# jonassibbesen/rpvg

Measured on AMD Instinct MI355X. Metric: read-pairs quantified/sec, higher is better.
Workload: dtype f64

## Files before the change

### include/rpvg_hip.h

```cpp
#ifndef RPVG_HIP_H
#define RPVG_HIP_H

#include <stdint.h>

#include "rpvg_batch.h"
#include "rpvg_rows.h"
#include "rpvg_index.h"
#include "rpvg_table.h"
#include "rpvg_samples.h"
#include "rpvg_text.h"

#ifdef __cplusplus
extern "C" {
#endif

typedef enum rpvg_hip_status {
    RPVG_HIP_OK = 0,
    RPVG_HIP_ERR_NO_DEVICE = -1,
    RPVG_HIP_ERR_RUNTIME = -2,
    RPVG_HIP_ERR_INVALID = -3,
    RPVG_HIP_ERR_ALLOC = -4,
    RPVG_HIP_ERR_UNSUPPORTED = -5
} rpvg_hip_status;

// ... 241 lines not shown
    const double * abundances;
    const double * noise_count;
    const double * total_count;
    const uint32_t * iterations;
    const uint32_t * set_count;
    const double * cluster_noise_count;
    const uint32_t * set_size;
    const uint32_t * set_member;
    const double * set_posterior;
    const double * set_abundance;
    const uint32_t * sample_count;
    const uint64_t * words_consumed;
    const uint32_t * generator_state;
} rpvg_hip_subset_em_independent_view;

typedef struct rpvg_independent_limits {
    uint32_t max_group_size;
    uint32_t max_samples;
    uint64_t max_transcript_sets;
    uint32_t words_per_draw;
    uint32_t state_words;
    uint64_t max_work_bytes;
} rpvg_independent_limits;

typedef struct rpvg_hip_independent_stats {
    uint64_t calls_completed;
    uint64_t draws;
    uint64_t subsets;
} rpvg_hip_independent_stats;

int rpvg_hip_nested_independent_subset_em(rpvg_hip_ctx * ctx, const rpvg_hip_batch * batch, const rpvg_hip_groups * groups,
                                          const rpvg_hip_independent_spec * spec, rpvg_hip_subset_em ** result_out);
int rpvg_hip_subset_em_get_independent(const rpvg_hip_subset_em * result, rpvg_hip_subset_em_independent_view * view_out);
int rpvg_hip_independent_draws_get(const rpvg_hip_subset_em * result, uint32_t unit, uint32_t * draws_out);
void rpvg_hip_independent_limits(rpvg_independent_limits * limits_out);
int rpvg_hip_independent_stats_get(rpvg_hip_ctx * ctx, rpvg_hip_independent_stats * stats_out);

int rpvg_hip_min_path_cover(rpvg_hip_ctx * ctx, const rpvg_hip_batch * batch, uint32_t num_clusters,
                            const uint32_t * clusters, const uint64_t * cover_off, uint32_t * cover, uint32_t * cover_size);
int rpvg_hip_min_path_cover_any(rpvg_hip_ctx * ctx, const rpvg_hip_batch * batch, uint32_t num_clusters,
                                const uint32_t * clusters, const uint64_t * cover_off, uint32_t * cover, uint32_t * cover_size,
                                uint64_t grid_min_work, uint32_t * choice_order);
typedef struct rpvg_cover_limits {
    uint32_t workgroup_max_paths;
    uint32_t chunk_rounds;
    uint64_t default_grid_min_work;
    uint64_t grid_max_rows;
    uint64_t grid_max_entries;
    uint32_t pick_block;
    uint32_t pick_per_thread;
    uint32_t pick_max_blocks;
    uint32_t strike_block;
    uint32_t strike_max_blocks;
    uint32_t hist_max_paths;
} rpvg_cover_limits;
void rpvg_hip_cover_limits(rpvg_cover_limits * limits_out);

int rpvg_hip_path_clusters(rpvg_hip_ctx * ctx, uint32_t num_paths, uint64_t num_sets, const uint64_t * set_off,
                           const uint32_t * set_path, uint32_t * path_to_cluster, uint32_t * num_clusters_out,
                           uint64_t * cluster_off, uint32_t * cluster_paths);

typedef struct rpvg_hip_alignments rpvg_hip_alignments;
typedef struct rpvg_hip_read_rows rpvg_hip_read_rows;
int rpvg_hip_alignments_upload(rpvg_hip_ctx * ctx, const rpvg_alignment_batch * alignments, rpvg_hip_alignments ** out);
void rpvg_hip_alignments_free(rpvg_hip_ctx * ctx, rpvg_hip_alignments * alignments);
int rpvg_hip_read_rows_build(rpvg_hip_ctx * ctx, const rpvg_hip_alignments * alignments, const rpvg_row_params * params,
                             int32_t merge, rpvg_hip_read_rows ** rows_out);
int rpvg_hip_read_rows_to_batch(rpvg_hip_ctx * ctx, const rpvg_hip_read_rows * rows, rpvg_hip_batch ** batch_out);
int rpvg_hip_read_rows_sizes(rpvg_hip_ctx * ctx, const rpvg_hip_read_rows * rows, rpvg_cluster_batch * view);
int rpvg_hip_read_rows_view(rpvg_hip_ctx * ctx, rpvg_hip_read_rows * rows, rpvg_cluster_batch * view, double * build_ms,
                            double * merge_ms);
void rpvg_hip_read_rows_free(rpvg_hip_ctx * ctx, rpvg_hip_read_rows * rows);

int rpvg_hip_frag_length_fit(rpvg_hip_ctx * ctx, const uint32_t * counts, uint32_t n, int skew_normal, rpvg_frag_length_fit * out);
int rpvg_hip_frag_length_table(rpvg_hip_ctx * ctx, double loc, double scale, double shape, rpvg_hip_frag_table ** out);
int rpvg_hip_frag_length_table_get(rpvg_hip_ctx * ctx, const rpvg_hip_frag_table * table, double * log_prob_out);
void rpvg_hip_frag_length_table_free(rpvg_hip_ctx * ctx, rpvg_hip_frag_table * table);
int rpvg_hip_effective_lengths(rpvg_hip_ctx * ctx, double loc, double scale, double shape, const uint32_t * path_length, uint64_t n,
                               double * out);
int rpvg_hip_alignments_set_effective_lengths(rpvg_hip_ctx * ctx, rpvg_hip_alignments * alignments, double loc, double scale,
                                              double shape, const uint32_t * path_length, double * out);
int rpvg_hip_frag_length_eval(rpvg_hip_ctx * ctx, int what, const double * rows, uint64_t n, double * out);

int rpvg_hip_align_index_create(rpvg_hip_ctx * ctx, const rpvg_index_params * params, rpvg_hip_align_index ** index_out);
void rpvg_hip_align_index_free(rpvg_hip_ctx * ctx, rpvg_hip_align_index * index);
int rpvg_hip_align_index_add(rpvg_hip_ctx * ctx, rpvg_hip_align_index * index, const rpvg_fragment_lists * chunk);
int rpvg_hip_align_index_finish(rpvg_hip_ctx * ctx, rpvg_hip_align_index * index, const uint64_t * extra_set_off,
                                const uint32_t * extra_set_path, uint64_t num_extra_sets, rpvg_index_info * info);
int rpvg_hip_align_index_frag_counts(rpvg_hip_ctx * ctx, const rpvg_hip_align_index * index, uint32_t * counts_out);
int rpvg_hip_align_index_view(rpvg_hip_ctx * ctx, rpvg_hip_align_index * index, rpvg_index_view * view_out);
int rpvg_hip_align_index_alignments(rpvg_hip_ctx * ctx, const rpvg_hip_align_index * index, const double * path_effective_length,
                                    const uint32_t * path_source_count, rpvg_hip_alignments ** alignments_out);

int rpvg_hip_path_table_upload(rpvg_hip_ctx * ctx, const rpvg_path_table * table, rpvg_hip_path_table ** table_out);
void rpvg_hip_path_table_free(rpvg_hip_ctx * ctx, rpvg_hip_path_table * table);
int rpvg_hip_read_rows_to_batch_with_paths(rpvg_hip_ctx * ctx, const rpvg_hip_read_rows * rows, const rpvg_hip_align_index * index,
                                           const rpvg_hip_path_table * table, rpvg_hip_batch ** batch_out);
int rpvg_hip_batch_path_group_ids(rpvg_hip_ctx * ctx, const rpvg_hip_batch * batch, uint32_t * group_ids_out);
void rpvg_hip_name_groups_limits(rpvg_name_groups_limits * limits_out);
int rpvg_hip_align_index_name_groups(rpvg_hip_ctx * ctx, const rpvg_hip_align_index * index, const rpvg_hip_path_table * table,
                                     rpvg_hip_name_groups ** groups_out);
int rpvg_hip_name_groups_view(rpvg_hip_ctx * ctx, rpvg_hip_name_groups * groups, rpvg_name_groups_view * view_out);
void rpvg_hip_name_groups_free(rpvg_hip_ctx * ctx, rpvg_hip_name_groups * groups);
int rpvg_hip_align_index_alignments_collapsed(rpvg_hip_ctx * ctx, const rpvg_hip_align_index * index, const rpvg_hip_path_table * table,
                                              const rpvg_hip_name_groups * groups, rpvg_hip_alignments ** alignments_out);

int rpvg_hip_estimates_table_build(rpvg_hip_ctx * ctx, const rpvg_estimates_flat * estimates, uint32_t ploidy, rpvg_hip_estimates_table ** table_out);
int rpvg_hip_estimates_table_tpm(rpvg_hip_ctx * ctx, rpvg_hip_estimates_table * table, double denominator);
int rpvg_hip_estimates_table_view(rpvg_hip_ctx * ctx, rpvg_hip_estimates_table * table, rpvg_estimates_table_view * view_out);
void rpvg_hip_estimates_table_limits(rpvg_estimates_table_limits * limits_out);
void rpvg_hip_estimates_table_free(rpvg_hip_ctx * ctx, rpvg_hip_estimates_table * table);

int rpvg_hip_gibbs_table_build(rpvg_hip_ctx * ctx, const rpvg_gibbs_flat * samples, rpvg_hip_gibbs_table ** table_out);
int rpvg_hip_gibbs_table_view(rpvg_hip_ctx * ctx, rpvg_hip_gibbs_table * table, rpvg_gibbs_table_view * view_out);
int rpvg_hip_gibbs_table_rows(rpvg_hip_ctx * ctx, rpvg_hip_gibbs_table * table, uint64_t first_path, uint64_t num_paths, double * rows_out);
void rpvg_hip_gibbs_table_limits(rpvg_gibbs_table_limits * limits_out);
void rpvg_hip_gibbs_table_free(rpvg_hip_ctx * ctx, rpvg_hip_gibbs_table * table);
int rpvg_hip_gibbs_read_counts_resident(rpvg_hip_ctx * ctx, const rpvg_hip_batch * batch, const rpvg_hip_em_problems * problems,
                                        const double * init_abundances, const double * init_noise_count, const uint32_t * num_samples,
                                        const uint64_t * seeds, uint32_t gibbs_thin_its, double gamma, rpvg_hip_gibbs_samples ** samples_out);
int rpvg_hip_gibbs_samples_get(rpvg_hip_ctx * ctx, const rpvg_hip_gibbs_samples * samples, double * noise_samples, double * abundance_samples);
void rpvg_hip_gibbs_samples_free(rpvg_hip_ctx * ctx, rpvg_hip_gibbs_samples * samples);
int rpvg_hip_gibbs_table_build_resident(rpvg_hip_ctx * ctx, const rpvg_hip_gibbs_samples * samples, const rpvg_hip_em_problems * problems,
                                        uint32_t num_clusters, const uint64_t * cluster_path_off, const double * total_count,
                                        uint32_t num_gibbs_samples, rpvg_hip_gibbs_table ** table_out);

int rpvg_hip_gibbs_table_text(rpvg_hip_ctx * ctx, const rpvg_hip_gibbs_table * table, const rpvg_table_labels * labels, int32_t precision,
                              rpvg_hip_table_text ** text_out);
int rpvg_hip_estimates_table_text(rpvg_hip_ctx * ctx, const rpvg_hip_estimates_table * table, const rpvg_estimates_flat * estimates,
                                  const rpvg_table_labels * labels, int32_t kind, int32_t precision, rpvg_hip_table_text ** text_out);
int rpvg_hip_table_text_view(rpvg_hip_table_text * text, rpvg_table_text_view * view_out);
int rpvg_hip_table_text_get(rpvg_hip_table_text * text, uint64_t byte_begin, uint64_t byte_end, char * dst);
int rpvg_hip_table_text_guards(rpvg_hip_table_text * text, int32_t * intact_out);
void rpvg_hip_table_text_free(rpvg_hip_table_text * text);

#define RPVG_HIP_COMM_ID_BYTES 128
int rpvg_hip_comm_unique_id(uint8_t * id_out);
int rpvg_hip_comm_init(rpvg_hip_ctx * ctx, const uint8_t * id, int world_size, int rank);
int rpvg_hip_comm_destroy(rpvg_hip_ctx * ctx);
int rpvg_hip_comm_init_all(rpvg_hip_ctx * const * ctxs, int num_contexts);
int rpvg_hip_comm_allreduce_sum_f64(rpvg_hip_ctx * ctx, double * device_buf, uint64_t n);
int rpvg_hip_gather(rpvg_hip_ctx * ctx, const double * local_values, uint64_t local_count, const uint64_t * counts, double * all_values);

int rpvg_hip_synth_dense_cluster(rpvg_hip_ctx * ctx, uint64_t seed, uint64_t num_rows, uint32_t num_paths,
                                 double * device_matrix, uint64_t ld, double * device_counts);
int rpvg_hip_synth_dense_rows(rpvg_hip_ctx * ctx, uint64_t seed, uint64_t row_begin, uint64_t num_rows, uint32_t num_paths,
                              double * device_matrix, uint64_t ld, double * device_counts);

int rpvg_hip_synth_dense_cluster_batch(rpvg_hip_ctx * ctx, uint64_t seed, uint64_t num_rows, uint32_t num_paths,
                                       rpvg_hip_batch ** batch_out);

int rpvg_hip_debug_log(rpvg_hip_ctx * ctx, uint64_t n, const double * x, double * out, int32_t use_table);

#define RPVG_HIP_EM_KERNELS 12
typedef struct rpvg_hip_em_kernel_stats {
    double ms;
    uint64_t launches;
    uint64_t problems;
    uint64_t iterations;
    uint64_t max_iterations;
    double alg_bytes;
} rpvg_hip_em_kernel_stats;
const char * rpvg_hip_em_kernel_name(int index);

typedef struct rpvg_hip_kernel_stats {
    double em_sparse_ms;      uint64_t em_sparse_launches;   double em_sparse_alg_bytes;
    double em_dense_ms;       uint64_t em_dense_launches;    double em_dense_alg_bytes;
    double loglik_ms;         uint64_t loglik_launches;      double loglik_evals;
    double build_ms;          uint64_t build_launches;
    double h2d_ms;            double h2d_bytes;
    uint64_t em_iterations_total;
    double search_pairs_possible; double search_pairs_table; double search_pairs_kept;
    rpvg_hip_em_kernel_stats em_kernel[RPVG_HIP_EM_KERNELS];
    double collapse_ms;
    double busy_ms;
    double gibbs_ms;
    double search_tile_ms;    uint64_t search_tile_launches;
    uint64_t gibbs_calls_completed;
    uint64_t gibbs_count_grid_problems;
    uint64_t gibbs_count_grid_iterations;
    uint64_t cover_grid_problems;
    uint64_t cover_grid_rounds;
    uint64_t text_exact_cells;
    uint64_t nested_full_calls;
    uint64_t nested_full_sets;
    uint64_t nested_full_retained;
} rpvg_hip_kernel_stats;

int rpvg_hip_stats_get(rpvg_hip_ctx * ctx, rpvg_hip_kernel_stats * stats_out);
int rpvg_hip_stats_reset(rpvg_hip_ctx * ctx);
int rpvg_hip_stats_intervals(rpvg_hip_ctx * ctx, uint64_t capacity, double * start_ms, double * stop_ms, int32_t * family,
                             uint64_t * count_out);

#ifdef __cplusplus
}
#endif

#endif
```

### rpvg_amd/csrc/group_build.hip

```cpp

#include "common.hpp"
#include "group_build_plan.hpp"

#include <hipcub/hipcub.hpp>

#include <algorithm>
#include <memory>
#include <type_traits>

using namespace rpvg_hip_detail;
using namespace rpvg_group_build;

static_assert(rpvg_group_build::kCollapseMaxMatrices == rpvg_hip_detail::kCollapseMaxMatrices && kStatusOk == RPVG_HIP_OK &&
              kStatusInvalid == RPVG_HIP_ERR_INVALID, "group_build_plan.hpp restates these");

namespace {

template <int BLOCK>
__global__ __launch_bounds__(BLOCK) void partitionRowsKernel(
    const uint32_t num_matrices, const uint64_t * __restrict__ mat_row_off, const uint64_t * __restrict__ mat_row0,
    const uint64_t * __restrict__ mat_rows, const double * __restrict__ row_count, const double * __restrict__ row_noise,
    uint32_t * __restrict__ row_perm, double * __restrict__ count_out, double * __restrict__ noise_out,
    uint32_t * __restrict__ mat_fast, uint32_t * __restrict__ mat_mid, const uint32_t mid_min_rows) {
    __shared__ uint32_t class_base[kNumRowClasses];
    __shared__ uint32_t wave_count[BLOCK / 64][kNumRowClasses];
    const uint32_t m = blockIdx.x;
    if (m >= num_matrices) return;
    const uint32_t R = static_cast<uint32_t>(mat_rows[m]);
    const double * cnt = row_count + mat_row0[m];
    const double * nz = row_noise + mat_row0[m];
    const uint64_t out0 = mat_row_off[m];
    const int lane = threadIdx.x & 63, wave = threadIdx.x >> 6;
    if (threadIdx.x < kNumRowClasses) class_base[threadIdx.x] = 0;
    __syncthreads();
    for (uint32_t i = threadIdx.x; i < R; i += BLOCK) atomicAdd(&class_base[rowClass(cnt[i], nz[i], R >= mid_min_rows)], 1u);
    __syncthreads();
    if (threadIdx.x == 0) {
        uint32_t running = 0;
        for (uint32_t c = 0; c < kNumRowClasses; ++c) {
            const uint32_t n = class_base[c];
            class_base[c] = running;
            running += n;
            if (c == 0) mat_fast[m] = running;
            if (c + 2 == kNumRowClasses) mat_mid[m] = running;
        }
    }
    __syncthreads();
    for (uint32_t c0 = 0; c0 < R; c0 += BLOCK) {
        const uint32_t i = c0 + threadIdx.x;
        const bool in = i < R;
        const double c = in ? cnt[i] : 0.0, z = in ? nz[i] : 0.0;
        const uint32_t mine = in ? rowClass(c, z, R >= mid_min_rows) : kNumRowClasses;
        uint32_t rank = 0;
#pragma unroll
        for (uint32_t k = 0; k < kNumRowClasses; ++k) {
            const unsigned long long ballot = __ballot(mine == k);
            if (mine == k) rank = __popcll(ballot & ((1ull << lane) - 1ull));
            if (lane == 0) wave_count[wave][k] = __popcll(ballot);
        }
        __syncthreads();
        if (in) {
            uint32_t dest = class_base[mine] + rank;
            for (int w = 0; w < wave; ++w) dest += wave_count[w][mine];
            row_perm[out0 + dest] = i;
            count_out[out0 + dest] = c;
            noise_out[out0 + dest] = z;
        }
        __syncthreads();
        if (threadIdx.x < kNumRowClasses) {
            uint32_t added = 0;
            for (int w = 0; w < BLOCK / 64; ++w) added += wave_count[w][threadIdx.x];
            class_base[threadIdx.x] += added;
        }
        __syncthreads();
    }
}

__global__ __launch_bounds__(256) void groupsBuildKernel(
    const uint32_t num_items, const uint32_t * __restrict__ item_matrix, const uint32_t * __restrict__ item_chunk,
    const uint64_t * __restrict__ mat_val_off, const uint64_t * __restrict__ mat_row_off,
    const uint64_t * __restrict__ mat_row0, const uint64_t * __restrict__ mat_rows, const uint32_t * __restrict__ mat_cols,
    const uint64_t * __restrict__ mat_inc_off,
    const uint64_t * __restrict__ path_grp_off,
    const uint32_t * __restrict__ path_grp, const uint64_t * __restrict__ row_ent_off,
    const uint32_t * __restrict__ ent_path, const double * __restrict__ ent_prob, const double * __restrict__ row_noise,
    const uint32_t * __restrict__ row_perm, const int normalise, double * __restrict__ values, double * __restrict__ rowmax,
    uint64_t * __restrict__ collapse_key, uint32_t * __restrict__ collapse_row, uint64_t * __restrict__ collapse_mask) {
    if (blockIdx.x >= num_items) return;
    const uint32_t m = item_matrix[blockIdx.x];
    const uint64_t R = mat_rows[m], r0 = mat_row0[m];
    const uint32_t G = mat_cols[m];
    double * M = values + mat_val_off[m];
    double * rm = rowmax + mat_row_off[m];
    const uint64_t * pgo = path_grp_off + mat_inc_off[m];
    const uint64_t i = static_cast<uint64_t>(item_chunk[blockIdx.x]) * 256 + threadIdx.x;
    if (i < R) {
        const uint64_t r = r0 + row_perm[mat_row_off[m] + i];
        for (uint64_t e = row_ent_off[r]; e < row_ent_off[r + 1]; ++e) {
            const uint32_t p = ent_path[e];
            const double v = ent_prob[e];
            for (uint64_t x = pgo[p]; x < pgo[p + 1]; ++x) M[static_cast<uint64_t>(path_grp[x]) * R + i] += v;
        }
        double mx = 0.0;
        if (normalise) {
            double rowsum = 0.0;
            for (uint32_t g = 0; g < G; ++g) rowsum += M[static_cast<uint64_t>(g) * R + i];
            const double keep = 1 - row_noise[r];
            double key = collapseWeight(G) * row_noise[r];
            uint64_t pattern = 0;
            for (uint32_t g = 0; g < G; ++g) {
                double v = (M[static_cast<uint64_t>(g) * R + i] / rowsum) * keep;
                if (v != v) v = 0.0;
                M[static_cast<uint64_t>(g) * R + i] = v;
                mx = (g == 0) ? v : fmax(mx, v);
                key = fma(collapseWeight(g), v, key);
                if (g < 64 && v != 0.0) pattern |= 1ull << g;
            }
            if (collapse_key) {
                collapse_key[mat_row_off[m] + i] = collapseSortKey(m, key, mx);
                collapse_row[mat_row_off[m] + i] = static_cast<uint32_t>(mat_row_off[m] + i);
                collapse_mask[mat_row_off[m] + i] = pattern;
            }
        } else {
            for (uint32_t g = 0; g < G; ++g) {
                const double v = M[static_cast<uint64_t>(g) * R + i];
                mx = (g == 0) ? v : fmax(mx, v);
            }
        }
        rm[i] = mx;
    }
}

__global__ __launch_bounds__(256) void groupsBuildTileKernel(
    const uint32_t num_items, const uint32_t * __restrict__ item_matrix, const uint32_t * __restrict__ item_chunk,
    const uint64_t * __restrict__ mat_val_off, const uint64_t * __restrict__ mat_row_off,
    const uint64_t * __restrict__ mat_row0, const uint64_t * __restrict__ mat_rows, const uint32_t * __restrict__ mat_cols,
    const uint64_t * __restrict__ mat_inc_off, const uint64_t * __restrict__ path_grp_off,
    const uint32_t * __restrict__ path_grp, const uint64_t * __restrict__ row_ent_off,
    const uint32_t * __restrict__ ent_path, const double * __restrict__ ent_prob, const double * __restrict__ row_noise,
    const uint32_t * __restrict__ row_perm, const int normalise, double * __restrict__ values, double * __restrict__ rowmax,
    uint64_t * __restrict__ collapse_key, uint32_t * __restrict__ collapse_row, uint64_t * __restrict__ collapse_mask) {
    extern __shared__ double tile[];
    if (blockIdx.x >= num_items) return;
    const uint32_t m = item_matrix[blockIdx.x];
    const uint64_t R = mat_rows[m], r0 = mat_row0[m];
    const uint32_t G = mat_cols[m];
    const uint32_t Rc = tileRows(G);
    const uint64_t i0 = static_cast<uint64_t>(item_chunk[blockIdx.x]) * Rc;
    const uint32_t nrows = static_cast<uint32_t>(min(static_cast<uint64_t>(Rc), R - i0));
    const uint32_t Rs = Rc + 1;
    const uint32_t cells = G * Rc;
    for (uint32_t idx = threadIdx.x; idx < G * Rs; idx += blockDim.x) tile[idx] = 0.0;
    __syncthreads();
    const uint32_t t = threadIdx.x;
    if (t < nrows) {
        const uint64_t r = r0 + row_perm[mat_row_off[m] + i0 + t];
        const uint64_t * pgo = path_grp_off + mat_inc_off[m];
        const uint64_t e_end = row_ent_off[r + 1];
        for (uint64_t e = row_ent_off[r]; e < e_end; e += 4) {
            uint32_t p[4];
            double v[4];
            uint64_t x_begin[4], x_end[4];
#pragma unroll
            for (int k = 0; k < 4; ++k) {
                const bool in = e + k < e_end;
                p[k] = in ? ent_path[e + k] : 0u;
                v[k] = in ? ent_prob[e + k] : 0.0;
            }
#pragma unroll
            for (int k = 0; k < 4; ++k) {
                const bool in = e + k < e_end;
                x_begin[k] = in ? pgo[p[k]] : 0;
                x_end[k] = in ? pgo[p[k] + 1] : 0;
            }
            constexpr int kAhead = 8;
            uint32_t columns[4][kAhead];
#pragma unroll
            for (int j = 0; j < kAhead; ++j) {
#pragma unroll
                for (int k = 0; k < 4; ++k) columns[k][j] = x_begin[k] + j < x_end[k] ? path_grp[x_begin[k] + j] : 0u;
            }
#pragma unroll
            for (int k = 0; k < 4; ++k) {
#pragma unroll
                for (int j = 0; j < kAhead; ++j) {
                    if (x_begin[k] + j < x_end[k]) tile[columns[k][j] * Rs + t] += v[k];
                }
                for (uint64_t x = x_begin[k] + kAhead; x < x_end[k]; x += kAhead) {
                    uint32_t more[kAhead];
#pragma unroll
                    for (int j = 0; j < kAhead; ++j) more[j] = x + j < x_end[k] ? path_grp[x + j] : 0u;
#pragma unroll
                    for (int j = 0; j < kAhead; ++j) {
                        if (x + j < x_end[k]) tile[more[j] * Rs + t] += v[k];
                    }
                }
            }
        }
    }
    __syncthreads();
    uint32_t parts = 1;
    while (parts < 8 && 2 * parts * Rc <= blockDim.x) parts *= 2;
    const uint32_t row = threadIdx.x / parts, part = threadIdx.x % parts;
    if (row < Rc) {
        const bool valid = row < nrows;
        const uint64_t r = valid ? r0 + row_perm[mat_row_off[m] + i0 + row] : 0;
        double mx = 0.0;
        if (normalise) {
            double rowsum = 0.0;
            if (valid && part == 0) {
                for (uint32_t g = 0; g < G; ++g) rowsum += tile[g * Rs + row];
            }
            rowsum = __shfl(rowsum, static_cast<int>(threadIdx.x & 63u) - static_cast<int>(part));
            const double noise = valid ? row_noise[r] : 0.0;
            const double keep = 1 - noise;
            double key = part == 0 ? collapseWeight(G) * noise : 0.0;
            uint64_t pattern = 0;
            if (valid) {
                for (uint32_t g = part; g < G; g += parts) {
                    double v = (tile[g * Rs + row] / rowsum) * keep;
                    if (v != v) v = 0.0;
                    tile[g * Rs + row] = v;
                    mx = fmax(mx, v);
                    key = fma(collapseWeight(g), v, key);
                    if (g < 64 && v != 0.0) pattern |= 1ull << g;
                }
            }
// ... 313 lines not shown

    uint64_t word[kWordHeld];
    double prob[kWordHeld];
    bool tiny_entry = false;
#pragma unroll
    for (int k = 0; k < kWordHeld; ++k) {
        word[k] = 0;
        prob[k] = 0.0;
        if (static_cast<uint32_t>(k) < n) {
            word[k] = words[a.ent_path[e_begin + k]];
            prob[k] = a.ent_prob[e_begin + k];
            tiny_entry |= !(prob[k] == 0.0 || prob[k] >= 0x1p-400);
        }
    }
    double cells[kWordMaxColumns];
#pragma unroll
    for (uint32_t c = 0; c < kWordMaxColumns; ++c) cells[c] = 0.0;
#pragma unroll
    for (int k = 0; k < kWordHeld; ++k) {
        if (static_cast<uint32_t>(k) < longest) addEntryToCells(cells, blocks, word[k], prob[k]);
    }
    for (uint32_t k = kWordHeld; k < longest; ++k) {
        uint64_t w = 0;
        double v = 0.0;
        if (k < n) {
            w = words[a.ent_path[e_begin + k]];
            v = a.ent_prob[e_begin + k];
            tiny_entry |= !(v == 0.0 || v >= 0x1p-400);
        }
        addEntryToCells(cells, blocks, w, v);
    }

    double rowsum = 0.0;
    if (a.normalise) {
#pragma unroll
        for (uint32_t b = 0; b < kWordMaxColumns / 8; ++b) {
            if (b < blocks) {
#pragma unroll
                for (uint32_t j = 0; j < 8; ++j) rowsum += cells[8 * b + j];
            }
        }
    }
    const double keep = 1 - noise;
    constexpr double kSmall = 0x1p-400, kLarge = 0x1p400;
    const bool plain = __ballot(valid && a.normalise && (!(rowsum == 0.0 || (rowsum >= kSmall && rowsum <= kLarge)) || tiny_entry)) == 0ull;
    double reciprocal = 0.0;
    if (plain) {
        reciprocal = __builtin_amdgcn_rcp(rowsum);
        reciprocal = fma(reciprocal, fma(-rowsum, reciprocal, 1.0), reciprocal);
        reciprocal = fma(reciprocal, fma(-rowsum, reciprocal, 1.0), reciprocal);
    }
    double key = collapseWeight(G) * noise, mx = 0.0;
    uint32_t pattern_lo = 0, pattern_hi = 0;
    double * out = M + i;
    auto columns = [&](const uint32_t b, auto all_eight, auto plain_division) {
#pragma unroll
        for (uint32_t j = 0; j < 8; ++j) {
            const uint32_t c = 8 * b + j;
            if (decltype(all_eight)::value || c < G) {
                double value = cells[c];
                if (a.normalise) {
                    if (decltype(plain_division)::value) {
                        const double quotient = value * reciprocal;
                        value = fma(fma(-rowsum, quotient, value), reciprocal, quotient);
                    } else {
                        value = value / rowsum;
                    }
                    value *= keep;
                    if (value != value) value = 0.0;
                    key = fma(collapseWeight(c), value, key);
                    if (c < 32) pattern_lo |= value != 0.0 ? 1u << (c & 31u) : 0u;
                    else pattern_hi |= value != 0.0 ? 1u << (c & 31u) : 0u;
                }
                asm("v_max_f64 %0, %1, %2" : "=v"(mx) : "v"(mx), "v"(value));
                if (valid) out[static_cast<uint64_t>(j) * R] = value;
            }
        }
        out += 8 * R;
    };
#pragma unroll
    for (uint32_t b = 0; b < kWordMaxColumns / 8; ++b) {
        if (8 * b + 8 <= G) {
            if (plain) columns(b, std::true_type(), std::true_type()); else columns(b, std::true_type(), std::false_type());
        } else if (8 * b < G) {
            if (plain) columns(b, std::false_type(), std::true_type()); else columns(b, std::false_type(), std::false_type());
        }
    }
    if (valid) {
        a.rowmax[row_off + i] = mx;
        if (a.normalise && a.collapse_key) {
            a.collapse_key[row_off + i] = collapseSortKey(m, key, mx);
            a.collapse_row[row_off + i] = static_cast<uint32_t>(row_off + i);
            a.collapse_mask[row_off + i] = (static_cast<uint64_t>(pattern_hi) << 32) | pattern_lo;
        }
    }
}

__global__ __launch_bounds__(256) void zeroWideMatricesKernel(const uint32_t * __restrict__ item_matrix, const uint32_t * __restrict__ item_chunk,
                                                              const uint64_t * __restrict__ mat_val_off, const uint64_t * __restrict__ mat_rows,
                                                              const uint32_t * __restrict__ mat_cols, double * __restrict__ values) {
    const uint32_t m = item_matrix[blockIdx.x];
    const uint64_t R = mat_rows[m];
    const uint64_t row = static_cast<uint64_t>(item_chunk[blockIdx.x]) * 256 + threadIdx.x;
    if (row >= R) return;
    double * M = values + mat_val_off[m];
    const uint32_t G = mat_cols[m];
    for (uint32_t g = 0; g < G; ++g) M[static_cast<uint64_t>(g) * R + row] = 0.0;
}

}

__global__ __launch_bounds__(256) void gatherSourceColumnsKernel(const uint32_t num_matrices, const uint32_t * __restrict__ cluster,
                                                                 const uint64_t * __restrict__ cluster_src_off, const uint32_t * __restrict__ src_col_count,
                                                                 const uint32_t * __restrict__ src_col_end, const uint32_t * __restrict__ src_col_path,
                                                                 const uint64_t * __restrict__ group_off, const uint64_t * __restrict__ first_path,
                                                                 uint64_t * __restrict__ group_path_off, uint32_t * __restrict__ group_path,
                                                                 uint32_t * __restrict__ column_counts) {
    const uint32_t m = blockIdx.x;
    if (m >= num_matrices) return;
    const uint64_t slot0 = cluster_src_off[cluster[m]];
    const uint64_t g0 = group_off[m], p0 = first_path[m];
    const uint32_t G = static_cast<uint32_t>(group_off[m + 1] - g0), L = static_cast<uint32_t>(first_path[m + 1] - p0);
    if (threadIdx.x == 0 && m == 0) group_path_off[0] = 0;
    for (uint32_t c = threadIdx.x; c < G; c += 256) {
        group_path_off[g0 + c + 1] = p0 + src_col_end[slot0 + c];
        column_counts[g0 + c] = src_col_count[slot0 + c];
    }
    for (uint32_t x = threadIdx.x; x < L; x += 256) group_path[p0 + x] = src_col_path[slot0 + x];
}

__global__ __launch_bounds__(256) void singlePathColumnsKernel(const uint32_t num_matrices, const uint64_t * __restrict__ group_off,
                                                               uint64_t * __restrict__ group_path_off, uint32_t * __restrict__ group_path) {
    const uint32_t m = blockIdx.x;
    if (m >= num_matrices) return;
    const uint64_t g0 = group_off[m];
    const uint32_t G = static_cast<uint32_t>(group_off[m + 1] - g0);
    if (threadIdx.x == 0 && m == 0) group_path_off[0] = 0;
    for (uint32_t c = threadIdx.x; c < G; c += 256) {
        group_path_off[g0 + c + 1] = g0 + c + 1;
        group_path[g0 + c] = c;
    }
}

namespace {

struct ItemBuffers {
    DeviceBuffer<uint32_t> matrix, chunk;
};

struct BuildTemporaries {
    DeviceBuffer<uint64_t> inc_off, path_grp_off, group_off, group_path_off, num_paths;
    DeviceBuffer<uint32_t> path_grp, group_path, degree, cursor, cluster;
    ItemBuffers list_items, tile_items, mask_items, word_items;
    DeviceBuffer<uint64_t> mask_off, masks, first_path, word_off, path_words;
    DeviceBuffer<uint32_t> column_counts;
    DeviceBuffer<unsigned char> scan_tmp;
};

struct BuildState {
    rpvg_hip_ctx * ctx;
    const rpvg_hip_batch * batch;
    const rpvg_hip_group_spec * spec;
    Columns kind;
    bool collapse;
    const GroupBuildPlan & plan;
    rpvg_hip_groups * g;
    BuildTemporaries & tmp;
    hipStream_t st;
    hipError_t e;
    size_t scan_bytes = 0;
    bool ok(const hipError_t r) {
        if (e == hipSuccess) e = r;
        return e == hipSuccess;
    }
};

BuildKnobs readBuildKnobs() {
    BuildKnobs knobs;
    const char * masks_env = std::getenv("RPVG_HIP_BUILD_MASKS");
    knobs.masks = masks_env ? std::atoi(masks_env) != 0 : true;
    knobs.words = masks_env ? std::atoi(masks_env) >= 2 : true;
    knobs.direct = !std::getenv("RPVG_HIP_NO_DIRECT_BUILD");
    return knobs;
}

void uploadPlan(BuildState & s) {
    const GroupBuildPlan & p = s.plan;
    const uint32_t M = p.M;
    rpvg_hip_groups * g = s.g;
    BuildTemporaries & t = s.tmp;
    UploadPack & pack = g->uploads;
    const auto addItems = [&pack](ItemBuffers & to, const Items & from) {
        pack.add(to.matrix, from.matrix.data(), from.size());
        pack.add(to.chunk, from.chunk.data(), from.size());
    };
    pack.add(g->mat_val_off, p.val_off.data(), M);
    pack.add(g->mat_row_off, p.row_off.data(), M);
    pack.add(g->mat_row0, p.row0.data(), M);
    pack.add(g->mat_rows, p.rows.data(), M);
    pack.add(g->mat_cols, p.cols.data(), M);
    pack.add(t.inc_off, p.inc_off.data(), M);
    pack.add(t.num_paths, p.num_paths.data(), M);
    pack.add(t.group_off, s.spec->group_off, M + 1);
    if (s.kind == Columns::Sources) {
        pack.add(t.first_path, s.spec->group_path_off, M + 1);
    } else if (s.kind == Columns::Lists) {
        pack.add(t.group_path_off, s.spec->group_path_off, p.num_columns + 1);
        pack.add(t.group_path, s.spec->group_path, p.num_incidences);
    }
    if (!p.list_items.empty()) addItems(t.list_items, p.list_items);
    if (!p.tile_items.empty()) addItems(t.tile_items, p.tile_items);
    if (!p.mask_items.empty()) {
        addItems(t.mask_items, p.mask_items);
        pack.add(t.mask_off, p.mask_off.data(), M);
    }
    if (!p.word_items.empty()) {
        addItems(t.word_items, p.word_items);
        pack.add(t.word_off, p.word_off.data(), M);
        pack.addZero(t.path_words, p.word_total);
    }
    pack.add(t.cluster, s.spec->cluster, M);
    if (p.lists_needed) {
        pack.addZero(t.degree, p.inc_total);
        pack.addZero(t.cursor, p.inc_total);
    }
    pack.addZero(g->build_error_flag, 1);
    s.ok(pack.commit(s.st));
}

void queueDeviceColumns(BuildState & s) {
    const GroupBuildPlan & p = s.plan;
    rpvg_hip_groups * g = s.g;
    BuildTemporaries & t = s.tmp;
    if (s.kind != Columns::Lists) {
        s.ok(t.group_path_off.alloc(p.num_columns + 1));
        s.ok(t.group_path.alloc(p.num_incidences));
    }
    if (s.kind == Columns::Sources) {
        s.ok(t.column_counts.alloc(p.num_columns));
        if (s.e == hipSuccess) {
            gatherSourceColumnsKernel<<<dim3(p.gather_columns.grid), dim3(p.gather_columns.block), 0, s.st>>>(
                p.M, t.cluster.ptr, s.batch->cluster_src_off.ptr, s.batch->src_col_count.ptr, s.batch->src_col_end.ptr, s.batch->src_col_path.ptr,
                t.group_off.ptr, t.first_path.ptr, t.group_path_off.ptr, t.group_path.ptr, t.column_counts.ptr);
            s.ok(hipGetLastError());
        }
        g->d_column_counts = t.column_counts.ptr;
    }
    if (s.kind == Columns::SinglePaths && s.e == hipSuccess) {
        singlePathColumnsKernel<<<dim3(p.single_path_columns.grid), dim3(p.single_path_columns.block), 0, s.st>>>(
            p.M, t.group_off.ptr, t.group_path_off.ptr, t.group_path.ptr);
        s.ok(hipGetLastError());
    }
    g->d_group_off = t.group_off.ptr;
    g->d_group_path_off = t.group_path_off.ptr;
    g->d_group_path = t.group_path.ptr;
    g->d_cluster = t.cluster.ptr;
}

void allocate(BuildState & s) {
    const GroupBuildPlan & p = s.plan;
    rpvg_hip_groups * g = s.g;
    BuildTemporaries & t = s.tmp;
    s.ok(g->values.alloc(p.val_total + 2));
    s.ok(g->rowmax.alloc(p.row_total));
    s.ok(g->row_perm.alloc(p.row_total));
    s.ok(g->row_count.alloc(p.row_total + 2));
    s.ok(g->row_noise.alloc(p.row_total + 2));
    s.ok(g->mat_fast.alloc(p.M));
    s.ok(g->mat_mid.alloc(p.M));
    if (s.collapse) {
        s.ok(g->collapse_key.alloc(p.row_total));
        s.ok(g->collapse_row.alloc(p.row_total));
        s.ok(g->collapse_mask.alloc(p.row_total));
    }
    if (p.lists_needed) {
        s.ok(t.path_grp_off.alloc(p.inc_total));
        s.ok(t.path_grp.alloc(p.num_incidences));
        if (s.e == hipSuccess) {
            s.ok(hipcub::DeviceScan::ExclusiveSum(nullptr, s.scan_bytes, t.degree.ptr, t.path_grp_off.ptr, static_cast<int>(p.inc_total), s.st));
        }
        s.ok(t.scan_tmp.alloc(s.scan_bytes));
        if (s.e == hipSuccess && p.inc_total > 0x7fffffffull) s.e = hipErrorInvalidValue;
    }
    if (!p.mask_items.empty()) s.ok(t.masks.alloc(p.mask_total));
}

void queueZeroWide(BuildState & s) {
    const GroupBuildPlan & p = s.plan;
    if (p.zero_wide.grid == 0) return;
    zeroWideMatricesKernel<<<dim3(p.zero_wide.grid), dim3(p.zero_wide.block), 0, s.st>>>(
        s.tmp.list_items.matrix.ptr, s.tmp.list_items.chunk.ptr, s.g->mat_val_off.ptr, s.g->mat_rows.ptr, s.g->mat_cols.ptr, s.g->values.ptr);
}

void queuePartition(BuildState & s) {
    const GroupBuildPlan & p = s.plan;
    rpvg_hip_groups * g = s.g;
    partitionRowsKernel<kPartitionThreads><<<dim3(p.partition.grid), dim3(p.partition.block), 0, s.st>>>(
        p.M, g->mat_row_off.ptr, g->mat_row0.ptr, g->mat_rows.ptr, s.batch->row_count.ptr, s.batch->row_noise.ptr, g->row_perm.ptr, g->row_count.ptr,
        g->row_noise.ptr, g->mat_fast.ptr, g->mat_mid.ptr, kMidMinRows);
}

MaskBuildArgs waveKernelArgs(const BuildState & s, const ItemBuffers & items, const uint64_t * set_off, const uint64_t * sets) {
    const rpvg_hip_groups * g = s.g;
    MaskBuildArgs a;
    memset(&a, 0, sizeof(a));
    a.num_items = static_cast<uint32_t>(items.matrix.count);
    a.item_matrix = items.matrix.ptr;
    a.item_chunk = items.chunk.ptr;
    a.mat_val_off = g->mat_val_off.ptr;
    a.mat_row_off = g->mat_row_off.ptr;
    a.mat_row0 = g->mat_row0.ptr;
    a.mat_rows = g->mat_rows.ptr;
    a.mat_cols = g->mat_cols.ptr;
    a.num_paths = s.tmp.num_paths.ptr;
    a.mask_off = set_off;
    a.masks = sets;
    a.row_ent_off = s.batch->row_ent_off.ptr;
    a.ent_path = s.batch->ent_path.ptr;
    a.ent_prob = s.batch->ent_prob.ptr;
    a.row_noise = s.batch->row_noise.ptr;
    a.row_perm = g->row_perm.ptr;
    a.normalise = s.spec->normalise ? 1 : 0;
#ifdef RPVG_HIP_EXPERIMENTS
    a.debug_no_long_rows = RPVG_EXPERIMENT_ENV("RPVG_HIP_BUILD_DEBUG") ? std::atoi(RPVG_EXPERIMENT_ENV("RPVG_HIP_BUILD_DEBUG")) & 1 : 0;
#endif
    a.values = g->values.ptr;
    a.rowmax = g->rowmax.ptr;
    a.collapse_key = g->collapse_key.ptr;
    a.collapse_row = g->collapse_row.ptr;
    a.collapse_mask = g->collapse_mask.ptr;
    return a;
}

void queueDirectRoute(BuildState & s) {
    const Launch & l = s.plan.build_single_paths;
    if (l.grid == 0) return;
    groupsBuildSinglePathKernel<<<dim3(l.grid), dim3(l.block), 0, s.st>>>(waveKernelArgs(s, s.tmp.mask_items, nullptr, nullptr));
}

void queueMaskRoute(BuildState & s) {
    const GroupBuildPlan & p = s.plan;
    BuildTemporaries & t = s.tmp;
    if (p.build_masks.grid == 0) return;
    columnMaskKernel<<<dim3(p.column_masks.grid), dim3(p.column_masks.block), 0, s.st>>>(
        p.M, p.num_columns, t.group_off.ptr, t.group_path_off.ptr, t.group_path.ptr, t.num_paths.ptr, t.mask_off.ptr, t.masks.ptr,
        s.g->build_error_flag.ptr);
    groupsBuildMaskKernel<<<dim3(p.build_masks.grid), dim3(p.build_masks.block), 0, s.st>>>(waveKernelArgs(s, t.mask_items, t.mask_off.ptr, t.masks.ptr));
}

void queueWordRoute(BuildState & s) {
    const GroupBuildPlan & p = s.plan;
    BuildTemporaries & t = s.tmp;
    if (p.build_words.grid == 0) return;
    pathColumnWordKernel<<<dim3(p.path_words.grid), dim3(p.path_words.block), 0, s.st>>>(
        p.M, p.num_columns, t.group_off.ptr, t.group_path_off.ptr, t.group_path.ptr, t.num_paths.ptr, t.word_off.ptr,
        reinterpret_cast<unsigned long long *>(t.path_words.ptr), s.g->build_error_flag.ptr);
    groupsBuildWordKernel<<<dim3(p.build_words.grid), dim3(p.build_words.block), 0, s.st>>>(
        waveKernelArgs(s, t.word_items, t.word_off.ptr, t.path_words.ptr));
}

void queueIncidenceInversion(BuildState & s) {
    const GroupBuildPlan & p = s.plan;
    BuildTemporaries & t = s.tmp;
    if (!p.lists_needed) return;
    incidenceCountKernel<<<dim3(p.incidence_count.grid), dim3(p.incidence_count.block), 0, s.st>>>(
        p.M, p.num_columns, t.group_off.ptr, t.group_path_off.ptr, t.group_path.ptr, t.inc_off.ptr, t.num_paths.ptr, t.degree.ptr,
        s.g->build_error_flag.ptr);
    s.ok(hipcub::DeviceScan::ExclusiveSum(t.scan_tmp.ptr, s.scan_bytes, t.degree.ptr, t.path_grp_off.ptr, static_cast<int>(p.inc_total), s.st));
    incidenceFillKernel<<<dim3(p.incidence_fill.grid), dim3(p.incidence_fill.block), 0, s.st>>>(
        p.M, p.num_columns, t.group_off.ptr, t.group_path_off.ptr, t.group_path.ptr, t.inc_off.ptr, t.num_paths.ptr, t.path_grp_off.ptr,
        t.cursor.ptr, t.path_grp.ptr);
}

using ListKernel = decltype(&groupsBuildKernel);
void queueListKernel(BuildState & s, const ListKernel kernel, const Launch & l, const ItemBuffers & items) {
    if (l.grid == 0) return;
    const rpvg_hip_groups * g = s.g;
    const BuildTemporaries & t = s.tmp;
    kernel<<<dim3(l.grid), dim3(l.block), l.lds_bytes, s.st>>>(
        static_cast<uint32_t>(items.matrix.count), items.matrix.ptr, items.chunk.ptr, g->mat_val_off.ptr, g->mat_row_off.ptr, g->mat_row0.ptr,
        g->mat_rows.ptr, g->mat_cols.ptr, t.inc_off.ptr, t.path_grp_off.ptr, t.path_grp.ptr, s.batch->row_ent_off.ptr, s.batch->ent_path.ptr,
        s.batch->ent_prob.ptr, s.batch->row_noise.ptr, g->row_perm.ptr, s.spec->normalise ? 1 : 0, g->values.ptr, g->rowmax.ptr,
        g->collapse_key.ptr, g->collapse_row.ptr, g->collapse_mask.ptr);
}
void queueTileRoute(BuildState & s) { queueListKernel(s, groupsBuildTileKernel, s.plan.build_tiles, s.tmp.tile_items); }
void queueListRoute(BuildState & s) { queueListKernel(s, groupsBuildKernel, s.plan.build_lists, s.tmp.list_items); }

void queueCollapse(BuildState & s) {
    rpvg_hip_ctx * ctx = s.ctx;
    rpvg_hip_groups * g = s.g;
    hipStream_t collapse_stream = ctx->collapse_stream;
    static const bool same_stream = RPVG_EXPERIMENT_ENV("RPVG_HIP_COLLAPSE_INLINE") != nullptr;
    if (same_stream) collapse_stream = s.st;
    s.ok(hipEventCreateWithFlags(&g->built, hipEventDisableTiming));
    s.ok(hipEventCreateWithFlags(&g->collapse_done, hipEventDisableTiming));
    if (s.e == hipSuccess && collapse_stream != s.st) {
        s.ok(hipEventRecord(g->built, s.st));
        s.ok(hipStreamWaitEvent(collapse_stream, g->built, 0));
    }
    const int collapse_span = (s.e == hipSuccess) ? ctx->spanBegin(FAM_COLLAPSE, collapse_stream) : -1;
    const char * before_env = std::getenv("RPVG_HIP_COLLAPSE_BEFORE_SEARCH");
    const bool before_search = before_env != nullptr && std::atoi(before_env) != 0;
    if (s.e == hipSuccess) {
        s.ok(queueRowCollapse(ctx, g, s.plan.row_total, s.spec->collapse_precision, collapse_stream, s.kind == Columns::Sources && !before_search));
    }
    ctx->spanEnd(collapse_span);
    if (s.e == hipSuccess) s.ok(hipEventRecord(g->collapse_done, collapse_stream));
}

int buildGroups(rpvg_hip_ctx * ctx, const rpvg_hip_batch * batch, const rpvg_hip_group_spec * spec, const Columns kind, rpvg_hip_groups ** groups_out) {
    RPVG_REQUIRE(spec->collapse_precision >= 0 && spec->collapse_precision < 1, "rpvg_hip_groups_build: collapse_precision outside [0, 1)");
    RPVG_REQUIRE(spec->collapse_precision == 0 || spec->normalise,
                 "rpvg_hip_groups_build: the row collapse applies to normalised matrices (src/path_abundance_estimator.cpp:379-380,442-443)");
    static const bool no_collapse = RPVG_EXPERIMENT_ENV("RPVG_HIP_NO_COLLAPSE") != nullptr;
    const bool collapse = spec->collapse_precision > 0 && !no_collapse;

    std::unique_ptr<rpvg_hip_groups> g(new (std::nothrow) rpvg_hip_groups());
    if (!g) {
        setError("rpvg_hip_groups_build: out of host memory");
        return RPVG_HIP_ERR_ALLOC;
    }
    g->batch = batch;
    g->num_matrices = spec->num_matrices;
    g->normalise = spec->normalise;

    std::unique_ptr<HostScope> scope_host(new HostScope("groups_build: host sizes"));
    GroupBuildPlan plan = planGroupBuild(batch->h_cluster_row_off.data(), batch->h_cluster_path_off.data(), batch->h_src_max_col_paths.data(),
                                         batch->num_clusters, spec->num_matrices, spec->cluster, spec->group_off, spec->group_path_off,
                                         spec->normalise != 0, collapse, kind, readBuildKnobs());
    if (plan.status != kStatusOk) {
        setError("%s", plan.message.c_str());
        return plan.status;
    }
    g->h_num_cols = plan.cols;
    g->h_num_rows = plan.rows;
    g->h_max_col_paths = std::move(plan.max_col_paths);
    g->h_num_paths = std::move(plan.paths);
    g->h_cluster = std::move(plan.cluster);
    if (plan.M == 0) {
        *groups_out = g.release();
        return RPVG_HIP_OK;
    }

    scope_host.reset();
    HostScope scope_dev("groups_build: upload + kernels + sync");
    std::lock_guard<std::mutex> lock(ctx->mutex);
    std::shared_ptr<BuildTemporaries> tmp = std::make_shared<BuildTemporaries>();
    BuildState s{ctx, batch, spec, kind, collapse, plan, g.get(), *tmp, ctx->stream, hipSetDevice(ctx->device)};
    g->build_temporaries.emplace_back(tmp);
    std::unique_ptr<HostScope> sub(new HostScope("groups_build: uploads"));
    int span = ctx->spanBegin(FAM_H2D);
    uploadPlan(s);
    queueDeviceColumns(s);
    ctx->spanEnd(span);
    ctx->stats.h2d_bytes += plan.h2d_bytes;
    sub.reset(new HostScope("groups_build: allocations"));
    allocate(s);
    sub.reset(new HostScope("groups_build: launches"));
    if (s.e == hipSuccess) {
        span = ctx->spanBegin(FAM_BUILD);
        queueZeroWide(s);
        queuePartition(s);
        queueDirectRoute(s);
        queueMaskRoute(s);
        queueWordRoute(s);
        queueIncidenceInversion(s);
        queueTileRoute(s);
        queueListRoute(s);
        sub.reset(new HostScope("groups_build: row collapse launches"));
        if (collapse && s.e == hipSuccess) queueCollapse(s);
        sub.reset();
        ctx->spanEnd(span);
        ctx->stats.build_launches += 3;
        s.ok(hipGetLastError());
        static const bool wait_here = RPVG_EXPERIMENT_ENV("RPVG_HIP_BUILD_SYNC") != nullptr;
        if (wait_here) s.ok(hipStreamSynchronize(s.st));
    }
    if (s.e != hipSuccess) {
        setError("rpvg_hip_groups_build: %s", hipGetErrorString(s.e));
        (void) hipStreamSynchronize(s.st);
        g.reset();
        return (s.e == hipErrorOutOfMemory) ? RPVG_HIP_ERR_ALLOC : RPVG_HIP_ERR_RUNTIME;
    }
    *groups_out = g.release();
    return RPVG_HIP_OK;
}

}

extern "C" int rpvg_hip_groups_build(rpvg_hip_ctx * ctx, const rpvg_hip_batch * batch, const rpvg_hip_group_spec * spec,
                                     rpvg_hip_groups ** groups_out) {
    RPVG_REQUIRE(ctx && batch && spec && groups_out, "rpvg_hip_groups_build: NULL argument");
    *groups_out = nullptr;
    RPVG_REQUIRE(spec->num_matrices == 0 || (spec->cluster && spec->group_off && spec->group_path_off && spec->group_path),
                 "rpvg_hip_groups_build: NULL spec arrays");
    return buildGroups(ctx, batch, spec, Columns::Lists, groups_out);
}

template <typename Sizes>
static int buildImpliedGroups(rpvg_hip_ctx * ctx, const rpvg_hip_batch * batch, const uint32_t num_matrices, const uint32_t * clusters, const int32_t normalise,
                              const double collapse_precision, const Columns kind, rpvg_hip_groups ** groups_out, const Sizes sizes) {
    std::vector<uint64_t> group_off(num_matrices + 1, 0), first_path(num_matrices + 1, 0);
    for (uint32_t m = 0; m < num_matrices; ++m) {
        const bool known = clusters[m] < batch->num_clusters;
        group_off[m + 1] = group_off[m] + (known ? sizes(clusters[m]).first : 0);
        first_path[m + 1] = first_path[m] + (known ? sizes(clusters[m]).second : 0);
    }
    rpvg_hip_group_spec spec;
    spec.num_matrices = num_matrices;
    spec.cluster = clusters;
    spec.group_off = group_off.data();
    spec.group_path_off = first_path.data();
    spec.group_path = nullptr;
    spec.normalise = normalise;
    spec.collapse_precision = collapse_precision;
    return buildGroups(ctx, batch, &spec, kind, groups_out);
}

extern "C" int rpvg_hip_groups_build_from_sources(rpvg_hip_ctx * ctx, const rpvg_hip_batch * batch, uint32_t num_matrices, const uint32_t * clusters,
                                                  int32_t normalise, double collapse_precision, rpvg_hip_groups ** groups_out) {
    RPVG_REQUIRE(ctx && batch && groups_out && (clusters || num_matrices == 0), "rpvg_hip_groups_build_from_sources: NULL argument");
    *groups_out = nullptr;
    if (!batch->has_source_columns) {
        setError("rpvg_hip_groups_build_from_sources: not taken (the batch was uploaded without PathInfo::source_ids, or their id ranges "
                 "outgrew the device scratch)");
        return RPVG_HIP_ERR_UNSUPPORTED;
    }
    for (uint32_t m = 0; m < num_matrices && clusters[m] < batch->num_clusters; ++m) {
        RPVG_REQUIRE(batch->h_src_num_cols[clusters[m]] > 0, "rpvg_hip_groups_build_from_sources: cluster %u has no source (haplotype) ids on its paths",
                     clusters[m]);
    }
    return buildImpliedGroups(ctx, batch, num_matrices, clusters, normalise, collapse_precision, Columns::Sources, groups_out, [batch](const uint32_t k) {
        return std::pair<uint64_t, uint64_t>(batch->h_src_num_cols[k], batch->h_src_col_paths[k]);
    });
}

extern "C" int rpvg_hip_groups_build_single_paths(rpvg_hip_ctx * ctx, const rpvg_hip_batch * batch, uint32_t num_matrices, const uint32_t * clusters,
                                                  int32_t normalise, double collapse_precision, rpvg_hip_groups ** groups_out) {
    RPVG_REQUIRE(ctx && batch && groups_out && (clusters || num_matrices == 0), "rpvg_hip_groups_build_single_paths: NULL argument");
    *groups_out = nullptr;
    return buildImpliedGroups(ctx, batch, num_matrices, clusters, normalise, collapse_precision, Columns::SinglePaths, groups_out, [batch](const uint32_t k) {
        const uint64_t paths = batch->h_cluster_path_off[k + 1] - batch->h_cluster_path_off[k];
        return std::pair<uint64_t, uint64_t>(paths, paths);
    });
}

int rpvg_hip_groups::buildError(hipStream_t stream) const {
    if (build_checked || !build_error_flag.ptr) return RPVG_HIP_OK;
    uint32_t bad = 0;
    hipError_t e = hipMemcpyAsync(&bad, build_error_flag.ptr, sizeof(uint32_t), hipMemcpyDeviceToHost, stream);
    if (e == hipSuccess) e = hipStreamSynchronize(stream);
    if (e != hipSuccess) {
        setError("rpvg_hip_groups_build: %s", hipGetErrorString(e));
        return RPVG_HIP_ERR_RUNTIME;
    }
    if (bad) {
        setError(bad == 2 ? "rpvg_hip_groups_build: a group lists a path twice" : "rpvg_hip_groups_build: a group refers to a path outside its cluster");
        return RPVG_HIP_ERR_INVALID;
    }
    build_checked = true;
    return RPVG_HIP_OK;
}

extern "C" void rpvg_hip_groups_free(rpvg_hip_ctx * ctx, rpvg_hip_groups * groups) {
    if (!groups) return;
    if (ctx) {
        std::lock_guard<std::mutex> lock(ctx->mutex);
        (void) hipSetDevice(ctx->device);
        (void) hipStreamSynchronize(ctx->stream);
        static const bool trace = std::getenv("RPVG_AMD_TRACE") != nullptr;
        if (trace && groups->collapse_info.ptr && groups->waitCollapse(ctx->stream) == hipSuccess) {
            uint32_t info[4] = {0, 0, 0, 0};
            if (hipMemcpyAsync(info, groups->collapse_info.ptr, sizeof(info), hipMemcpyDeviceToHost, ctx->stream) == hipSuccess &&
                hipStreamSynchronize(ctx->stream) == hipSuccess) {
                std::fprintf(stderr, "[rpvg_hip trace]   row collapse: %u of %u matrices replayed (%u sorted whole), %u active rows, %u rows took their head's values\n",
                             info[0], groups->num_matrices, info[2], info[3], info[1]);
            }
        }
        delete groups;
    } else {
        delete groups;
    }
}
```

### rpvg_amd/csrc/group_build_plan.hpp

```cpp
#ifndef RPVG_GROUP_BUILD_PLAN_HPP
#define RPVG_GROUP_BUILD_PLAN_HPP

#include <algorithm>
#include <cstddef>
#include <cstdint>
#include <cstdio>
#include <string>
#include <vector>

#ifndef RPVG_PLAN_FN
#if defined(__HIPCC__)
#define RPVG_PLAN_FN __host__ __device__ inline
#else
#define RPVG_PLAN_FN inline
#endif
#endif

namespace rpvg_group_build {

constexpr uint32_t kTileDoubles = 4096;

RPVG_PLAN_FN uint32_t tileRows(const uint32_t G) {
    if (G * 16u > kTileDoubles) return 0;
    uint32_t rows = 256;
    while (rows * G > kTileDoubles) rows >>= 1;
    return rows;
}

constexpr uint32_t kMaskMaxColumns = 1024;
constexpr uint32_t kMaskMaxWords = 16;
constexpr uint32_t kMaskRows = 64;
constexpr uint32_t kWordMaxColumns = 64;
constexpr uint32_t kListRows = 256;

constexpr uint32_t kTileLdsBytes = (kTileDoubles + 256) * sizeof(double);
constexpr uint32_t kPartitionThreads = 1024;

constexpr uint32_t kCollapseMaxMatrices = 1u << 20;
constexpr int kStatusOk = 0, kStatusInvalid = -3;

enum class Columns {
    Lists,
    Sources,
    SinglePaths,
};

struct BuildKnobs {
    bool masks = true;
    bool words = true;
    bool direct = true;
};

struct Launch {
    uint32_t grid = 0, block = 0, lds_bytes = 0;
};

struct Items {
    std::vector<uint32_t> matrix, chunk;
    size_t size() const { return matrix.size(); }
    bool empty() const { return matrix.empty(); }
    void add(const uint32_t m, const uint64_t rows, const uint32_t rows_per_item) {
        for (uint64_t c = 0; c * rows_per_item < rows; ++c) {
            matrix.push_back(m);
            chunk.push_back(static_cast<uint32_t>(c));
        }
    }
};

struct GroupBuildPlan {
    int status = kStatusOk;
    std::string message;
    uint32_t M = 0;
    std::vector<uint64_t> val_off, row_off, row0, rows, inc_off, num_paths;
    std::vector<uint64_t> mask_off, word_off;
    std::vector<uint32_t> cols, max_col_paths, paths, cluster;
    uint64_t val_total = 0, row_total = 0, inc_total = 0, mask_total = 0, word_total = 0;
    Items list_items, tile_items, mask_items, word_items;
    bool lists_needed = false;
    bool direct = false;
    uint64_t num_columns = 0, num_incidences = 0;
    double h2d_bytes = 0;
    Launch gather_columns, single_path_columns;
    Launch zero_wide, partition;
    Launch build_single_paths, column_masks, build_masks;
    Launch path_words, build_words;
    Launch incidence_count, incidence_fill;
    Launch build_tiles, build_lists;
};

namespace detail {
template <typename... Args>
inline GroupBuildPlan refuse(const char * format, Args... args) {
    GroupBuildPlan p;
    char text[512];
    std::snprintf(text, sizeof(text), format, args...);
    p.status = kStatusInvalid;
    p.message = text;
    return p;
}
}

inline GroupBuildPlan planGroupBuild(const uint64_t * h_cluster_row_off, const uint64_t * h_cluster_path_off, const uint32_t * h_src_max_col_paths,
                                     const uint32_t num_clusters, const uint32_t M, const uint32_t * cluster, const uint64_t * group_off,
                                     const uint64_t * group_path_off, const bool normalise, const bool collapse, const Columns kind,
                                     const BuildKnobs & knobs) {
    GroupBuildPlan p;
    p.M = M;
    p.direct = kind == Columns::SinglePaths && !normalise && knobs.direct;
    for (auto * v : {&p.val_off, &p.row_off, &p.row0, &p.rows, &p.inc_off, &p.num_paths}) v->assign(M, 0);
    p.mask_off.assign(M, ~0ull);
    p.word_off.assign(M, ~0ull);
    p.cols.assign(M, 0);
    for (uint32_t m = 0; m < M; ++m) {
        const uint32_t k = cluster[m];
        if (k >= num_clusters) return detail::refuse("rpvg_hip_groups_build: matrix %u refers to cluster %u of %u", m, k, num_clusters);
        const uint64_t R = h_cluster_row_off[k + 1] - h_cluster_row_off[k];
        const uint64_t N = h_cluster_path_off[k + 1] - h_cluster_path_off[k];
        const uint64_t g0 = group_off[m], g1 = group_off[m + 1];
        if (R > 0xffffffffull) {
            return detail::refuse("rpvg_hip_groups_build: matrix %u has %llu rows (limit 2^32 - 1)", m, static_cast<unsigned long long>(R));
        }
        if (R == 0 || g1 <= g0) return detail::refuse("rpvg_hip_groups_build: matrix %u has no rows or no columns", m);
        p.rows[m] = R;
        p.cols[m] = static_cast<uint32_t>(g1 - g0);
        uint64_t longest = 0;
        if (kind == Columns::Sources) longest = h_src_max_col_paths[k];
        else if (kind == Columns::SinglePaths) longest = 1;
        else for (uint64_t c = g0; c < g1; ++c) longest = std::max<uint64_t>(longest, group_path_off[c + 1] - group_path_off[c]);
        p.max_col_paths.push_back(static_cast<uint32_t>(std::min<uint64_t>(longest, 0xffffffffu)));
        p.paths.push_back(static_cast<uint32_t>(N));
        p.cluster.push_back(k);
        p.row0[m] = h_cluster_row_off[k];
        p.num_paths[m] = N;
        p.val_off[m] = p.val_total;
        p.row_off[m] = p.row_total;
        p.inc_off[m] = p.inc_total;
        p.val_total += R * (g1 - g0);
        p.row_total += R;
        p.inc_total += N + 1;
        const uint64_t mask_words = (N + 63) / 64;
        if (p.direct) {
            p.mask_items.add(m, R, kMaskRows);
        } else if (knobs.words && p.cols[m] <= kWordMaxColumns) {
            p.word_off[m] = p.word_total;
            p.word_total += N;
            p.word_items.add(m, R, kMaskRows);
        } else if (knobs.masks && p.cols[m] <= kMaskMaxColumns && mask_words <= kMaskMaxWords) {
            p.mask_off[m] = p.mask_total;
            p.mask_total += p.cols[m] * mask_words;
            p.mask_items.add(m, R, kMaskRows);
        } else {
            p.lists_needed = true;
            const uint32_t tile_rows = tileRows(p.cols[m]);
            if (tile_rows) p.tile_items.add(m, R, tile_rows);
            else p.list_items.add(m, R, kListRows);
        }
    }
    if (collapse && (M >= kCollapseMaxMatrices || p.row_total > 0x7fffffffull)) {
        return detail::refuse("rpvg_hip_groups_build: the row collapse takes up to %u matrices and 2^31 - 1 rows per call (got %u matrices, %llu rows): "
                              "build the matrices of a batch in several calls", kCollapseMaxMatrices - 1, M, static_cast<unsigned long long>(p.row_total));
    }
    if (M == 0) return p;
    p.num_columns = group_off[M];
    p.num_incidences = kind == Columns::Lists ? group_path_off[p.num_columns] : group_path_off[M];
    p.h2d_bytes = static_cast<double>(M * 60 + p.num_columns * 8 + p.num_incidences * 4 + (p.list_items.size() + p.tile_items.size()) * 8);

    const auto items = [](const Items & list) { return static_cast<uint32_t>(list.size()); };
    const auto waves = [](const Items & list) { return list.empty() ? Launch{} : Launch{(static_cast<uint32_t>(list.size()) + 3) / 4, 256, 0}; };
    const uint32_t col_blocks = static_cast<uint32_t>((p.num_columns + 255) / 256);
    const Launch per_column{col_blocks, 256, 0}, per_matrix{M, 256, 0};
    if (kind == Columns::Sources) p.gather_columns = per_matrix;
    if (kind == Columns::SinglePaths) p.single_path_columns = per_matrix;
    if (!p.list_items.empty()) p.zero_wide = p.build_lists = Launch{items(p.list_items), kListRows, 0};
    p.partition = Launch{M, kPartitionThreads, 0};
    if (p.direct) {
        p.build_single_paths = waves(p.mask_items);
    } else if (!p.mask_items.empty()) {
        p.column_masks = per_column;
        p.build_masks = waves(p.mask_items);
    }
    if (!p.word_items.empty()) {
        p.path_words = per_column;
        p.build_words = waves(p.word_items);
    }
    if (p.lists_needed) p.incidence_count = p.incidence_fill = per_column;
    if (!p.tile_items.empty()) p.build_tiles = Launch{items(p.tile_items), 256, kTileLdsBytes};
    return p;
}

}

#endif
```

### rpvg_amd/csrc/subset_em.hip

```cpp

#include "common.hpp"
#include "subset_pack.hpp"

#include <cmath>
#include <memory>

using namespace rpvg_hip_detail;

namespace {

constexpr uint32_t kMaxSelected = 1024;

struct MergedList {
    const uint32_t * a;
    const uint32_t * b;
    uint32_t na, nb, i, j;
    __device__ __forceinline__ MergedList(const uint32_t * a_in, uint32_t na_in, const uint32_t * b_in, uint32_t nb_in)
        : a(a_in), b(b_in), na(na_in), nb(nb_in), i(0), j(0) {}
    __device__ __forceinline__ bool done() const { return i >= na && j >= nb; }
    __device__ __forceinline__ uint32_t next() {
        if (j >= nb || (i < na && a[i] <= b[j])) return a[i++];
        return b[j++];
    }
};
// ... 183 lines not shown
            const uint32_t path = walk.next();
            distinct += (path != previous) ? 1u : 0u;
            previous = path;
        }
        args.slot_first[slot0 + rank] = first[sel[s]];
        args.slot_second[slot0 + rank] = second[sel[s]];
        args.slot_weight[slot0 + rank] = weight[s];
        args.slot_length[slot0 + rank] = length[s];
        args.slot_columns[slot0 + rank] = distinct;
        my_subsets += 1;
        my_length += length[s];
        my_columns += distinct;
    }
    if (my_subsets) {
        atomicAdd(&red[0], my_subsets);
        atomicAdd(&red[1], my_length);
        atomicAdd(&red[2], my_columns);
    }
    __syncthreads();
    if (threadIdx.x == 0) {
        const uint64_t r0 = args.cluster_row_off[k], r1 = args.cluster_row_off[k + 1];
        const unsigned long long rows = r1 - r0, entries = args.row_ent_off[r1] - args.row_ent_off[r0];
        *out_totals = MatrixTotals{red[0], red[1], red[2], red[0] * rows, red[0] * entries, red[0] * ((rows + args.segment_rows - 1) / args.segment_rows)};
    }
}

__global__ __launch_bounds__(64) void subsetSelectSmallKernel(const SelectArgs args) {
    const uint32_t m = blockIdx.x;
    if (m >= args.num_matrices) return;
    if (args.pair_count[m] > kSmallSelected) {
        if (threadIdx.x == 0) args.big_matrices[atomicAdd(&args.header->big_count, 1u)] = m;
        return;
    }
    selectSubsetsOfMatrix<kSmallSelected, kSmallCachedPaths, 64>(args, m);
}

__global__ __launch_bounds__(256) void subsetSelectWideKernel(const SelectArgs args) {
    const uint32_t count = args.header->big_count;
    for (uint32_t item = blockIdx.x; item < count; item += gridDim.x) {
        selectSubsetsOfMatrix<kMaxSelected, kWideCachedPaths, 256>(args, args.big_matrices[item]);
        __syncthreads();
    }
}

struct ExpandArgs {
    uint32_t num_matrices;
    const SubsetHeader * header;
    const MatrixTotals * totals;
    const MatrixTotals * bases;
    const uint64_t * slot_off;
    const uint32_t * slot_first;
    const uint32_t * slot_second;
    const double * slot_weight;
    const uint32_t * slot_length;
    const uint32_t * slot_columns;
    const uint64_t * group_off;
    const uint64_t * group_path_off;
    const uint32_t * group_path;
    const uint32_t * cluster;
    const uint64_t * cluster_row_off;
    const uint64_t * row_ent_off;
    uint32_t * sub_cluster;
    double * sub_weight;
    uint64_t * path_off;
    uint32_t * path;
    uint64_t * col_off;
    uint32_t * col_path;
    uint64_t * row_base;
    uint64_t * ent_base;
    uint64_t * seg_first;
    uint32_t * item_problem;
    uint32_t segment_rows;
    uint64_t * subset_off;
};

__global__ __launch_bounds__(256) void subsetExpandKernel(const ExpandArgs args) {
    constexpr int BLOCK = 256;
    __shared__ uint32_t scratch[BLOCK / 64];
    const uint32_t m = blockIdx.x;
    if (m >= args.num_matrices) return;
    const MatrixTotals base = args.bases[m];
    if (threadIdx.x == 0) {
        args.subset_off[m] = args.header->overflow ? 0 : base.subsets;
        if (m + 1 == args.num_matrices) args.subset_off[m + 1] = args.header->overflow ? 0 : args.header->subsets;
    }
    if (args.header->overflow) return;
    const uint32_t n = static_cast<uint32_t>(args.totals[m].subsets);
    const uint64_t slot0 = args.slot_off[m];
    const Columns columns{args.group_path_off, args.group_path, args.group_off[m]};
    const uint32_t k = args.cluster[m];
    const uint64_t r0 = args.cluster_row_off[k], r1 = args.cluster_row_off[k + 1];
    const uint64_t rows = r1 - r0, entries = args.row_ent_off[r1] - args.row_ent_off[r0];
    uint64_t length_run = base.list_length, columns_run = base.columns;
    for (uint32_t c = 0; c < n; c += BLOCK) {
        const uint32_t r = c + threadIdx.x;
        const uint32_t len = r < n ? args.slot_length[slot0 + r] : 0u, cols = r < n ? args.slot_columns[slot0 + r] : 0u;
        uint32_t len_total, cols_total;
        const uint32_t len_before = blockExclusiveScan<BLOCK>(len, len_total, scratch);
        const uint32_t cols_before = blockExclusiveScan<BLOCK>(cols, cols_total, scratch);
        if (r < n) {
            const uint64_t s = base.subsets + r;
            const uint64_t p0 = length_run + len_before, c0 = columns_run + cols_before;
            args.sub_cluster[s] = k;
            args.sub_weight[s] = args.slot_weight[slot0 + r];
            args.path_off[s] = p0;
            args.col_off[s] = c0;
            args.row_base[s] = base.rows + static_cast<uint64_t>(r) * rows;
            args.ent_base[s] = base.entries + static_cast<uint64_t>(r) * entries;
            const uint64_t segments = (rows + args.segment_rows - 1) / args.segment_rows, item0 = base.segments + static_cast<uint64_t>(r) * segments;
            args.seg_first[s] = item0;
            for (uint64_t item = item0; item < item0 + segments; ++item) args.item_problem[item] = static_cast<uint32_t>(s);
            MergedList list = columns.list(args.slot_first[slot0 + r], args.slot_second[slot0 + r]);
            uint32_t previous = 0xffffffffu;
            uint64_t pw = p0, cw = c0;
            while (!list.done()) {
                const uint32_t path = list.next();
                args.path[pw++] = path;
                if (path != previous) args.col_path[cw++] = path;
                previous = path;
            }
        }
        length_run += len_total;
        columns_run += cols_total;
    }
}

constexpr uint32_t kMergeLdsRecords = 2048;
constexpr unsigned long long kMergeNoRecord = ~0ull;
constexpr uint32_t kMergePathBits = 27, kMergeRankBits = 10;

struct MergeArgs {
    const SubsetHeader * header;
    uint32_t num_matrices;
    const uint64_t * subset_off;
    const double * weight;
    const uint64_t * path_off;
    const uint32_t * path;
    const uint64_t * col_off;
    const uint32_t * col_path;
    const double * abundances;
    const double * noise;
    const double * total;
    const uint32_t * cluster;
    const uint64_t * cluster_path_off;
    const uint32_t * path_group_id;
    unsigned long long * sort_key;
    uint32_t * sort_pos;
    double * rec_a0;
    double * rec_a1;
    uint32_t * merge_bad;
    unsigned char * packed;
};

__global__ __launch_bounds__(256) void subsetMergeKernel(const MergeArgs args) {
    constexpr int BLOCK = 256;
    __shared__ unsigned long long s_key[kMergeLdsRecords];
    __shared__ uint32_t s_pos[kMergeLdsRecords];
    __shared__ uint32_t s_scan[BLOCK / 64];
    const SubsetHeader h = *args.header;
    if (h.overflow) return;
    const uint32_t m = blockIdx.x, tid = threadIdx.x;
    const uint64_t M = args.num_matrices;
    if (m >= M) return;
    const PackedLayout lay = packedLayout(M, h.subsets, h.list_length, h.columns);
    uint32_t * set_count = reinterpret_cast<uint32_t *>(args.packed + lay.set_count);
    double * cluster_noise = reinterpret_cast<double *>(args.packed + lay.cluster_noise);
    uint32_t * set_first = reinterpret_cast<uint32_t *>(args.packed + lay.set_first);
    uint32_t * set_second = reinterpret_cast<uint32_t *>(args.packed + lay.set_second);
    double * set_posterior = reinterpret_cast<double *>(args.packed + lay.set_posterior);
    double * set_abund = reinterpret_cast<double *>(args.packed + lay.set_abund);
    const uint64_t s0 = args.subset_off[m];
    const uint32_t n = static_cast<uint32_t>(args.subset_off[m + 1] - s0);
    if (n == 0) {
        if (tid == 0) {
            set_count[m] = 0;
            cluster_noise[m] = 0.0;
        }
        return;
    }
    const uint64_t base = args.path_off[s0];
    const uint32_t Lm = static_cast<uint32_t>(args.path_off[s0 + n] - base);
    const uint32_t * gid = args.path_group_id + args.cluster_path_off[args.cluster[m]];
    if (tid == BLOCK - 1) {
        double noise = 0.0, sum_hap_prob = 0.0;
        for (uint32_t r = 0; r < n; ++r) {
            const double w = args.weight[s0 + r];
            sum_hap_prob = addRounded(sum_hap_prob, w);
            noise = addRounded(noise, mulRounded(args.noise[s0 + r], w));
        }
        cluster_noise[m] = addRounded(noise, mulRounded(addRounded(1.0, -sum_hap_prob), args.total[s0]));
    }
    uint32_t P2 = 2;
    while (P2 < Lm) P2 <<= 1;
    unsigned long long * keys = s_key;
    uint32_t * order = s_pos;
    if (P2 > kMergeLdsRecords) {
        keys = args.sort_key + 2 * base;
        order = args.sort_pos + 2 * base;
    }
    for (uint32_t pos = tid; pos < P2; pos += BLOCK) {
        unsigned long long key = kMergeNoRecord;
        if (pos < Lm) {
            uint32_t lo = 0, hi = n - 1;
            while (lo < hi) {
                const uint32_t mid = (lo + hi + 1) >> 1;
                if (args.path_off[s0 + mid] - base <= pos) lo = mid; else hi = mid - 1;
            }
            const uint32_t r = lo;
            const uint32_t l0 = static_cast<uint32_t>(args.path_off[s0 + r] - base), L = static_cast<uint32_t>(args.path_off[s0 + r + 1] - base) - l0;
            const uint32_t * list = args.path + base + l0;
            const uint32_t j = pos - l0;
            const uint32_t g = gid[list[j]];
            uint32_t members = 0, first = 0, second = 0;
            for (uint32_t t = 0; t < L; ++t) {
                if (gid[list[t]] == g) {
                    if (members == 0) first = t;
                    else if (members == 1) second = t;
                    ++members;
                }
            }
            if (members > 2) *args.merge_bad = 1;
            if (first == j && members <= 2) {
                const uint32_t p0 = list[first], p1 = (members == 2) ? list[second] : 0xffffffffu;
                const double w = args.weight[s0 + r];
                const uint64_t c0 = args.col_off[s0 + r];
                const uint32_t C = static_cast<uint32_t>(args.col_off[s0 + r + 1] - c0);
                const uint32_t * cols = args.col_path + c0;
                auto column = [&](const uint32_t p) {
                    uint32_t a = 0, b = C;
                    while (a < b) {
                        const uint32_t mid = (a + b) >> 1;
                        if (cols[mid] < p) a = mid + 1; else b = mid;
                    }
                    return a;
                };
                const double multiplicity = (members == 2 && p0 == p1) ? 2.0 : 1.0;
                args.rec_a0[base + pos] = mulRounded(args.abundances[c0 + column(p0)], w) / multiplicity;
                args.rec_a1[base + pos] = (members == 2) ? mulRounded(args.abundances[c0 + column(p1)], w) / multiplicity : 0.0;
                key = (static_cast<unsigned long long>(p0 + 1) << (kMergePathBits + kMergeRankBits)) |
                      (static_cast<unsigned long long>(members == 2 ? p1 + 1 : 0u) << kMergeRankBits) | r;
            }
        }
        keys[pos] = key;
        order[pos] = pos;
    }
    __syncthreads();
    for (uint32_t k2 = 2; k2 <= P2; k2 <<= 1) {
        for (uint32_t j2 = k2 >> 1; j2 > 0; j2 >>= 1) {
            for (uint32_t i = tid; i < P2; i += BLOCK) {
                const uint32_t x = i ^ j2;
                if (x > i) {
                    const unsigned long long a = keys[i], b = keys[x];
                    if ((a > b) == ((i & k2) == 0)) {
                        keys[i] = b;
                        keys[x] = a;
                        const uint32_t oa = order[i];
                        order[i] = order[x];
                        order[x] = oa;
                    }
                }
            }
            __syncthreads();
        }
    }
    uint32_t Q = 0;
    for (uint32_t c0 = 0; c0 < Lm; c0 += BLOCK) {
        const uint32_t i = c0 + tid;
        const unsigned long long key = i < Lm ? keys[i] : kMergeNoRecord;
        const bool start = key != kMergeNoRecord && (i == 0 || (keys[i - 1] >> kMergeRankBits) != (key >> kMergeRankBits));
        uint32_t total;
        const uint32_t before = blockExclusiveSum<BLOCK>(start ? 1u : 0u, total, s_scan);
        if (start) {
            const unsigned long long set = key >> kMergeRankBits;
            double posterior = 0.0, a0 = 0.0, a1 = 0.0;
            for (uint32_t e = i; e < Lm && keys[e] != kMergeNoRecord && (keys[e] >> kMergeRankBits) == set; ++e) {
                const uint32_t r = static_cast<uint32_t>(keys[e] & ((1u << kMergeRankBits) - 1u)), pos = order[e];
                posterior = addRounded(posterior, args.weight[s0 + r]);
                a0 = addRounded(a0, args.rec_a0[base + pos]);
                a1 = addRounded(a1, args.rec_a1[base + pos]);
            }
            const uint64_t q = base + Q + before;
            const uint32_t second = static_cast<uint32_t>(set & ((1u << kMergePathBits) - 1u));
            set_first[q] = static_cast<uint32_t>(set >> kMergePathBits) - 1;
            set_second[q] = second ? second - 1 : 0xffffffffu;
            set_posterior[q] = posterior;
            set_abund[2 * q] = a0;
            set_abund[2 * q + 1] = a1;
        }
        Q += total;
    }
    if (tid == 0) set_count[m] = Q;
}

}


static int nestedSubsetEmAttempt(rpvg_hip_ctx * ctx, const rpvg_hip_batch * batch, const rpvg_hip_groups * groups,
                                 const uint32_t * column_counts, double min_rel_likelihood, double min_hap_prob,
                                 uint32_t max_em_its, double max_rel_em_conv, double collapse_precision,
                                 rpvg_hip_subset_em ** result_out, bool * did_not_fit, PairSearchWork & search, const bool second_attempt) {
    *did_not_fit = false;
    RPVG_REQUIRE(min_rel_likelihood > 0, "rpvg_hip_nested_subset_em: min_rel_likelihood must be positive");
    RPVG_REQUIRE(max_em_its > 0, "rpvg_hip_nested_subset_em: max_em_its must be positive");
    RPVG_REQUIRE(groups->batch == batch, "rpvg_hip_nested_subset_em: the matrices were built on another batch");
    const uint32_t M = groups->num_matrices;
    RPVG_REQUIRE(M == 0 || column_counts || groups->d_column_counts, "rpvg_hip_nested_subset_em: column_counts is NULL");
    std::unique_ptr<rpvg_hip_subset_em> res(new (std::nothrow) rpvg_hip_subset_em());
    if (!res) {
        setError("rpvg_hip_nested_subset_em: out of host memory");
        return RPVG_HIP_ERR_ALLOC;
    }
    res->num_matrices = M;

    const bool disabled = std::getenv("RPVG_HIP_NO_DEVICE_SUBSETS") != nullptr;
    if (disabled || !(min_hap_prob * kMaxSelected >= 1.0)) {
        setError("rpvg_hip_nested_subset_em: not taken (min_hap_prob %g admits more than %u subsets per cluster, or RPVG_HIP_NO_DEVICE_SUBSETS)",
                 min_hap_prob, kMaxSelected);
        return RPVG_HIP_ERR_UNSUPPORTED;
    }
    std::unique_ptr<HostScope> scope(new HostScope("subset em: bounds"));
    uint64_t slots = 0, lane_rows = 0, lane_entries = 0, lane_paths = 0, max_cluster_work = 0;
    uint32_t max_paths = 0;
    std::vector<uint64_t> slot_off(M + 1, 0);
    for (uint32_t m = 0; m < M; ++m) {
        const uint64_t G = groups->h_num_cols[m];
        slot_off[m + 1] = slot_off[m] + std::min<uint64_t>(G * (G + 1) / 2, kMaxSelected);
        const uint32_t k = groups->h_cluster[m];
        lane_rows += batch->h_cluster_row_off[k + 1] - batch->h_cluster_row_off[k];
        lane_entries += batch->h_cluster_ent_off[k + 1] - batch->h_cluster_ent_off[k];
        lane_paths += groups->h_num_paths[m];
        max_paths = std::max(max_paths, groups->h_num_paths[m]);
        max_cluster_work = std::max<uint64_t>(max_cluster_work, (batch->h_cluster_row_off[k + 1] - batch->h_cluster_row_off[k]) +
                                                                    (batch->h_cluster_ent_off[k + 1] - batch->h_cluster_ent_off[k]));
    }
    slots = slot_off[M];
    if (M > 0 && 8ull * (5ull * (static_cast<uint64_t>(max_paths) + 1) + 6) > 156 * 1024) {
        setError("rpvg_hip_nested_subset_em: not taken (a cluster with %u paths: EM vectors in global memory)", max_paths);
        return RPVG_HIP_ERR_UNSUPPORTED;
    }

    std::lock_guard<std::mutex> lock(ctx->mutex);
    RPVG_HIP_CHECK(hipSetDevice(ctx->device));
    hipStream_t st = ctx->stream;
    if (M == 0) {
        *result_out = res.release();
        return RPVG_HIP_OK;
    }
    SubsetEmHints & hints = ctx->subset_hints;
    auto planned = [](const double per_unit, const unsigned long long units, const double headroom) {
        return static_cast<unsigned long long>(std::ceil(per_unit * headroom * static_cast<double>(units)));
    };
    unsigned long long cap_subsets = std::min<unsigned long long>(slots, hints.subsets_per_matrix > 0 ? planned(hints.subsets_per_matrix, M, 1.25) + 256 : std::max<unsigned long long>(8ull * M, 16384));
    unsigned long long cap_length = std::max<unsigned long long>(planned(hints.list_per_path, lane_paths, 2.0), std::max<unsigned long long>(8 * lane_paths, 1u << 20));
    unsigned long long cap_rows = hints.rows_per_row > 0 ? planned(hints.rows_per_row, lane_rows, 1.25) + 65536 : 8 * lane_rows;
    unsigned long long cap_entries = hints.entries_per_entry > 0 ? planned(hints.entries_per_entry, lane_entries, 1.25) + 65536 : 8 * lane_entries;
    if (hints.retry) {
        cap_subsets = std::min<unsigned long long>(slots, std::max(cap_subsets, hints.retry_subsets + 64));
        cap_length = std::max(cap_length, hints.retry_list_length + 64);
        cap_rows = std::max(cap_rows, hints.retry_rows + 64);
        cap_entries = std::max(cap_entries, hints.retry_entries + 64);
        hints.retry = false;
    }
    const unsigned long long cap_columns = cap_length;
    const unsigned long long cap_items = cap_rows / emFillSegmentRows() + cap_subsets;

    scope.reset(new HostScope("subset em: search + kernels queued"));
    const size_t header_room = 256;
    int rc = RPVG_HIP_OK;
    if (!second_attempt) {
        search.extra_u64 = slot_off.data();
        search.extra_u64_count = M + 1;
        search.extra_zero_bytes = header_room + emQueuesBytes();
        rc = queuePairSearch(ctx, groups, column_counts, min_rel_likelihood, search);
        if (rc != RPVG_HIP_OK) return rc;
    } else {
        const hipError_t zeroed = zeroAsync(search.d_extra_zero.ptr, search.extra_zero_bytes, st);
        if (zeroed != hipSuccess) {
            setError("rpvg_hip_nested_subset_em: %s", hipGetErrorString(zeroed));
            return RPVG_HIP_ERR_RUNTIME;
        }
    }

    hipError_t e = hipSuccess;
    auto ok = [&](hipError_t r) { if (e == hipSuccess) e = r; return e == hipSuccess; };
    const uint64_t * d_slot_off = search.d_extra_u64.ptr;
    SubsetHeader * header = reinterpret_cast<SubsetHeader *>(search.d_extra_zero.ptr);
    static_assert(sizeof(SubsetHeader) <= 256, "room for the header");
    DeviceBuffer<uint32_t> d_slot_first, d_slot_second, d_slot_length, d_slot_columns;
    DeviceBuffer<double> d_slot_weight;
    DeviceBuffer<unsigned char> d_totals, d_bases, d_packed;
    ok(d_slot_first.alloc(slots));
    ok(d_slot_second.alloc(slots));
    ok(d_slot_length.alloc(slots));
    ok(d_slot_columns.alloc(slots));
    ok(d_slot_weight.alloc(slots));
    ok(d_totals.alloc(sizeof(MatrixTotals) * M));
    ok(d_bases.alloc(sizeof(MatrixTotals) * M));
    DeviceBuffer<uint32_t> d_big_matrices;
    ok(d_big_matrices.alloc(M));
    DeviceBuffer<uint32_t> d_sub_cluster, d_path, d_col_path, d_iters, d_kept_rows, d_kept_entries;
    DeviceBuffer<double> d_sub_weight, d_abund, d_noise, d_total;
    DeviceBuffer<uint64_t> d_path_off, d_col_off, d_row_base, d_ent_base, d_subset_off, d_seg_first;
    DeviceBuffer<uint32_t> d_item_problem;
    ok(d_sub_cluster.alloc(cap_subsets));
    ok(d_sub_weight.alloc(cap_subsets));
    ok(d_path_off.alloc(cap_subsets + 1));
    ok(d_col_off.alloc(cap_subsets + 1));
    ok(d_row_base.alloc(cap_subsets));
    ok(d_ent_base.alloc(cap_subsets));
    ok(d_subset_off.alloc(M + 1));
    ok(d_seg_first.alloc(cap_subsets + 1));
    ok(d_item_problem.alloc(cap_items));
    ok(d_path.alloc(cap_length));
    ok(d_col_path.alloc(cap_columns));
    ok(d_abund.alloc(cap_columns));
    ok(d_noise.alloc(cap_subsets));
    ok(d_total.alloc(cap_subsets));
    ok(d_iters.alloc(cap_subsets));
    ok(d_kept_rows.alloc(cap_subsets));
    ok(d_kept_entries.alloc(cap_subsets));
    const size_t packed_capacity = packedLayout(M, cap_subsets, cap_length, cap_columns).bytes;
    ok(d_packed.alloc(packed_capacity));
    const bool merge_here = batch->path_group_id.ptr != nullptr && max_paths < (1u << kMergePathBits) - 2;
    DeviceBuffer<unsigned long long> d_merge_key;
    DeviceBuffer<uint32_t> d_merge_pos;
    DeviceBuffer<double> d_merge_a0, d_merge_a1;
    if (merge_here) {
        ok(d_merge_key.alloc(2 * cap_length + 2));
        ok(d_merge_pos.alloc(2 * cap_length + 2));
        ok(d_merge_a0.alloc(cap_length));
        ok(d_merge_a1.alloc(cap_length));
    }
    void * pinned_header = nullptr;
    if (e == hipSuccess && pinnedAlloc(&pinned_header, sizeof(SubsetHeader)) != hipSuccess) e = hipErrorOutOfMemory;
    hipEvent_t header_here = nullptr;
    if (e == hipSuccess) ok(hipEventCreateWithFlags(&header_here, hipEventDisableTiming));
    if (e != hipSuccess) {
        setError("rpvg_hip_nested_subset_em: %s", hipGetErrorString(e));
        (void) hipStreamSynchronize(st);
        leavePairSearch(ctx);
        if (pinned_header) pinnedFree(pinned_header);
        if (header_here) (void) hipEventDestroy(header_here);
        return (e == hipErrorOutOfMemory) ? RPVG_HIP_ERR_ALLOC : RPVG_HIP_ERR_RUNTIME;
    }
    MatrixTotals * totals = reinterpret_cast<MatrixTotals *>(d_totals.ptr);
    MatrixTotals * bases = reinterpret_cast<MatrixTotals *>(d_bases.ptr);

    std::unique_ptr<HostScope> part_scope(new HostScope("subset em: select + offsets + expand queued"));
    int span = ctx->spanBegin(FAM_BUILD);
    SelectArgs sa;
    sa.num_matrices = M;
    sa.pair_count = search.d_tail.ptr;
    sa.pair_cap_off = search.d_pair_cap_off.ptr;
    sa.pair_first = search.d_out_first.ptr;
    sa.pair_second = search.d_out_second.ptr;
    sa.pair_value = search.d_out_value.ptr;
    sa.group_off = groups->d_group_off;
    sa.group_path_off = groups->d_group_path_off;
    sa.group_path = groups->d_group_path;
    sa.cluster = groups->d_cluster;
    sa.mat_rows = groups->mat_rows.ptr;
    sa.cluster_row_off = batch->cluster_row_off.ptr;
    sa.row_ent_off = batch->row_ent_off.ptr;
    sa.slot_off = d_slot_off;
    sa.min_hap_prob = min_hap_prob;
    sa.segment_rows = emFillSegmentRows();
    sa.slot_first = d_slot_first.ptr;
    sa.slot_second = d_slot_second.ptr;
    sa.slot_weight = d_slot_weight.ptr;
    sa.slot_length = d_slot_length.ptr;
    sa.slot_columns = d_slot_columns.ptr;
    sa.totals = totals;
    sa.header = header;
    sa.big_matrices = d_big_matrices.ptr;
    subsetSelectSmallKernel<<<dim3(M), dim3(64), 0, st>>>(sa);
    subsetSelectWideKernel<<<dim3(std::min<uint32_t>(M, 128)), dim3(256), 0, st>>>(sa);
    const bool check_build = !groups->build_checked && groups->build_error_flag.ptr;
    OffsetsArgs oa;
    oa.pair_count = search.d_tail.ptr;
    oa.log_evals = reinterpret_cast<const unsigned long long *>(search.d_tail.ptr + search.evals_word);
    oa.build_error = check_build ? groups->build_error_flag.ptr : nullptr;
    oa.num_matrices = M;
    oa.totals = totals;
    oa.bases = bases;
    oa.header = header;
    oa.cap_subsets = cap_subsets;
    oa.cap_length = cap_length;
    oa.cap_columns = cap_columns;
    oa.cap_rows = cap_rows;
    oa.cap_entries = cap_entries;
    oa.cap_items = cap_items;
    oa.seg_first = d_seg_first.ptr;
    oa.path_off = d_path_off.ptr;
    oa.col_off = d_col_off.ptr;
    subsetOffsetsKernel<<<dim3(1), dim3(1024), 0, st>>>(oa);
    SubsetHeader * h_header = static_cast<SubsetHeader *>(pinned_header);
    ok(hipMemcpyAsync(h_header, header, sizeof(SubsetHeader), hipMemcpyDeviceToHost, st));
    ok(hipEventRecord(header_here, st));
    ExpandArgs ea;
    ea.num_matrices = M;
    ea.header = header;
    ea.totals = totals;
    ea.bases = bases;
    ea.slot_off = d_slot_off;
    ea.slot_first = d_slot_first.ptr;
    ea.slot_second = d_slot_second.ptr;
    ea.slot_weight = d_slot_weight.ptr;
    ea.slot_length = d_slot_length.ptr;
    ea.slot_columns = d_slot_columns.ptr;
    ea.group_off = groups->d_group_off;
    ea.group_path_off = groups->d_group_path_off;
    ea.group_path = groups->d_group_path;
    ea.cluster = groups->d_cluster;
    ea.cluster_row_off = batch->cluster_row_off.ptr;
    ea.row_ent_off = batch->row_ent_off.ptr;
    ea.sub_cluster = d_sub_cluster.ptr;
    ea.sub_weight = d_sub_weight.ptr;
    ea.path_off = d_path_off.ptr;
    ea.path = d_path.ptr;
    ea.col_off = d_col_off.ptr;
    ea.col_path = d_col_path.ptr;
    ea.row_base = d_row_base.ptr;
    ea.ent_base = d_ent_base.ptr;
    ea.seg_first = d_seg_first.ptr;
    ea.item_problem = d_item_problem.ptr;
    ea.segment_rows = emFillSegmentRows();
    ea.subset_off = d_subset_off.ptr;
    subsetExpandKernel<<<dim3(M), dim3(256), 0, st>>>(ea);
    ok(hipGetLastError());
    ctx->spanEnd(span);
    ctx->stats.build_launches += 4;
    leavePairSearch(ctx);

    part_scope.reset();
    EmProblemList list;
    list.P_bound = static_cast<uint32_t>(std::min<unsigned long long>(cap_subsets, 0xfffffffeull));
    list.d_num_problems = &header->num_problems;
    list.d_cluster = d_sub_cluster.ptr;
    list.d_col_off = d_col_off.ptr;
    list.d_col_path = d_col_path.ptr;
    list.d_row_base = d_row_base.ptr;
    list.d_ent_base = d_ent_base.ptr;
    list.rows_capacity = cap_rows;
    list.entries_capacity = cap_entries;
    list.d_seg_first = d_seg_first.ptr;
    list.d_item_problem = d_item_problem.ptr;
    list.items_bound = static_cast<uint32_t>(std::min<unsigned long long>(cap_items, 0xfffffffeull));
    list.d_num_items = &header->num_items;
    list.max_cols = max_paths + 1;
    list.max_cluster_paths = max_paths;
    list.max_cluster_work = max_cluster_work;
    list.wide_capacity = 0;
    EmOutputs out{d_abund.ptr, d_noise.ptr, d_iters.ptr, d_kept_rows.ptr, d_kept_entries.ptr, d_total.ptr};
    EmSolveWork work;
    work.zeroed_queues = search.d_extra_zero.ptr + header_room;
    if (e == hipSuccess) {
        rc = queueEmSolve(ctx, batch, list, max_em_its, max_rel_em_conv, out, work, collapse_precision);
        if (rc != RPVG_HIP_OK) {
            (void) hipStreamSynchronize(st);
            (void) hipEventDestroy(header_here);
            pinnedFree(pinned_header);
            return rc;
        }
    }
    part_scope.reset(new HostScope("subset em: merge + pack queued"));
    static_assert(sizeof(SubsetHeader) <= 192, "the merge's flag word sits behind the header");
    uint32_t * d_merge_bad = reinterpret_cast<uint32_t *>(search.d_extra_zero.ptr + 192);
    if (merge_here && e == hipSuccess) {
        MergeArgs ma;
        ma.header = header;
        ma.num_matrices = M;
        ma.subset_off = d_subset_off.ptr;
        ma.weight = d_sub_weight.ptr;
        ma.path_off = d_path_off.ptr;
        ma.path = d_path.ptr;
        ma.col_off = d_col_off.ptr;
        ma.col_path = d_col_path.ptr;
        ma.abundances = d_abund.ptr;
        ma.noise = d_noise.ptr;
        ma.total = d_total.ptr;
        ma.cluster = groups->d_cluster;
        ma.cluster_path_off = batch->cluster_path_off.ptr;
        ma.path_group_id = batch->path_group_id.ptr;
        ma.sort_key = d_merge_key.ptr;
        ma.sort_pos = d_merge_pos.ptr;
        ma.rec_a0 = d_merge_a0.ptr;
        ma.rec_a1 = d_merge_a1.ptr;
        ma.merge_bad = d_merge_bad;
        ma.packed = d_packed.ptr;
        const int merge_span = ctx->spanBegin(FAM_BUILD);
        subsetMergeKernel<<<dim3(M), dim3(256), 0, st>>>(ma);
        ctx->spanEnd(merge_span);
        ctx->stats.build_launches += 1;
    }
    PackArgs pa;
    pa.merge_bad = merge_here ? d_merge_bad : nullptr;
    pa.header = header;
    pa.num_matrices = M;
    pa.subset_off = d_subset_off.ptr;
    pa.weight = d_sub_weight.ptr;
    pa.path_off = d_path_off.ptr;
    pa.col_off = d_col_off.ptr;
    pa.abundances = d_abund.ptr;
    pa.noise = d_noise.ptr;
    pa.total = d_total.ptr;
    pa.path = d_path.ptr;
    pa.col_path = d_col_path.ptr;
    pa.iterations = d_iters.ptr;
    pa.kept_rows = d_kept_rows.ptr;
    pa.kept_entries = d_kept_entries.ptr;
    pa.packed = d_packed.ptr;
    packResultsKernel<<<dim3(256), dim3(256), 0, st>>>(pa);
    ok(hipGetLastError());

    part_scope.reset();
    scope.reset(new HostScope("subset em: header"));
    if (e == hipSuccess) ok(waitEvent(header_here));
    (void) hipEventDestroy(header_here);
    if (e != hipSuccess) {
        setError("rpvg_hip_nested_subset_em: %s", hipGetErrorString(e));
        (void) hipStreamSynchronize(st);
        pinnedFree(pinned_header);
        return (e == hipErrorOutOfMemory) ? RPVG_HIP_ERR_ALLOC : RPVG_HIP_ERR_RUNTIME;
    }
    const SubsetHeader got = *h_header;
    pinnedFree(pinned_header);
    {
        auto fold = [](double & kept, const unsigned long long needed, const unsigned long long units) {
            kept = std::max(0.9 * kept, static_cast<double>(needed) / static_cast<double>(std::max<unsigned long long>(units, 1)));
        };
        fold(hints.subsets_per_matrix, got.subsets, M);
        fold(hints.list_per_path, got.list_length, lane_paths);
        fold(hints.rows_per_row, got.rows, lane_rows);
        fold(hints.entries_per_entry, got.entries, lane_entries);
    }
    if (got.build_bad) {
        (void) hipStreamSynchronize(st);
        setError(got.build_bad == 2 ? "rpvg_hip_groups_build: a group lists a path twice" : "rpvg_hip_groups_build: a group refers to a path outside its cluster");
        return RPVG_HIP_ERR_INVALID;
    }
    groups->build_checked = true;
    if (got.overflow) {
        (void) hipStreamSynchronize(st);
        setError("rpvg_hip_nested_subset_em: not taken (%llu subsets, %llu rows, %llu entries, %llu selected-diplotype overflows: over the reserved "
                 "capacity)", got.subsets, got.rows, got.entries, got.select_overflow);
        if (!got.select_overflow) {
            hints.retry = true;
            hints.retry_subsets = got.subsets;
            hints.retry_list_length = std::max(got.list_length, got.columns);
            hints.retry_rows = got.rows;
            hints.retry_entries = got.entries;
            *did_not_fit = true;
        }
        return RPVG_HIP_ERR_UNSUPPORTED;
    }
    scope.reset(new HostScope("subset em: wait for the EM + download"));
    const uint64_t S = got.subsets;
    const PackedLayout lay = packedLayout(M, S, got.list_length, got.columns);
    if (pinnedAlloc(&res->block, std::max<size_t>(lay.bytes, 64)) != hipSuccess) {
        (void) hipStreamSynchronize(st);
        setError("rpvg_hip_nested_subset_em: out of page-locked host memory");
        return RPVG_HIP_ERR_ALLOC;
    }
    unsigned char * host = static_cast<unsigned char *>(res->block);
    ok(hipMemcpyAsync(host, d_packed.ptr, lay.bytes, hipMemcpyDeviceToHost, st));
    ok(waitStream(st));
    if (e != hipSuccess) {
        setError("rpvg_hip_nested_subset_em: %s", hipGetErrorString(e));
        return RPVG_HIP_ERR_RUNTIME;
    }
    accountPairSearch(ctx, groups, search, got.log_evals, got.kept_pairs);

    rpvg_hip_subset_em_view & v = res->view;
    v.num_matrices = M;
    v.subset_off = reinterpret_cast<const uint64_t *>(host + lay.subset_off);
    v.weight = reinterpret_cast<const double *>(host + lay.weight);
    v.path_off = reinterpret_cast<const uint64_t *>(host + lay.path_off);
    v.path = reinterpret_cast<const uint32_t *>(host + lay.path);
    v.col_off = reinterpret_cast<const uint64_t *>(host + lay.col_off);
    v.col_path = reinterpret_cast<const uint32_t *>(host + lay.col_path);
    v.abundances = reinterpret_cast<const double *>(host + lay.abundances);
    v.noise_count = reinterpret_cast<const double *>(host + lay.noise);
    v.total_count = reinterpret_cast<const double *>(host + lay.total);
    v.iterations = reinterpret_cast<const uint32_t *>(host + lay.iterations);
    if (merge_here) {
        if (*reinterpret_cast<const uint32_t *>(host + lay.merge_flags)) {
            setError("rpvg_hip_nested_subset_em: a diplotype's path subset holds more than two paths of one transcript (PathInfo::group_id): "
                     "the reference asserts against it (src/path_abundance_estimator.cpp:722)");
            return RPVG_HIP_ERR_INVALID;
        }
        v.set_count = reinterpret_cast<const uint32_t *>(host + lay.set_count);
        v.cluster_noise_count = reinterpret_cast<const double *>(host + lay.cluster_noise);
        v.set_first = reinterpret_cast<const uint32_t *>(host + lay.set_first);
        v.set_second = reinterpret_cast<const uint32_t *>(host + lay.set_second);
        v.set_posterior = reinterpret_cast<const double *>(host + lay.set_posterior);
        v.set_abundance = reinterpret_cast<const double *>(host + lay.set_abund);
    }
    res->num_subsets = S;
    accountEmSolve(ctx, static_cast<uint32_t>(S), v.col_off, reinterpret_cast<const uint32_t *>(host + lay.kept_rows),
                   reinterpret_cast<const uint32_t *>(host + lay.kept_entries), v.iterations);
    *result_out = res.release();
    return RPVG_HIP_OK;
}

extern "C" int rpvg_hip_nested_subset_em(rpvg_hip_ctx * ctx, const rpvg_hip_batch * batch, const rpvg_hip_groups * groups,
                                         const uint32_t * column_counts, double min_rel_likelihood, double min_hap_prob,
                                         uint32_t max_em_its, double max_rel_em_conv, double collapse_precision,
                                         rpvg_hip_subset_em ** result_out) {
    RPVG_REQUIRE(ctx && batch && groups && result_out, "rpvg_hip_nested_subset_em: NULL argument");
    *result_out = nullptr;
    bool did_not_fit = false;
    PairSearchWork search;
    int rc = nestedSubsetEmAttempt(ctx, batch, groups, column_counts, min_rel_likelihood, min_hap_prob, max_em_its, max_rel_em_conv, collapse_precision,
                                   result_out, &did_not_fit, search, false);
    if (rc == RPVG_HIP_ERR_UNSUPPORTED && did_not_fit) {
        static const bool trace = std::getenv("RPVG_AMD_TRACE") != nullptr;
        if (trace) std::fprintf(stderr, "[rpvg_hip trace]   subset em: second attempt (%s)\n", rpvg_hip_last_error());
        rc = nestedSubsetEmAttempt(ctx, batch, groups, column_counts, min_rel_likelihood, min_hap_prob, max_em_its, max_rel_em_conv, collapse_precision,
                                   result_out, &did_not_fit, search, true);
    }
    return rc;
}

extern "C" int rpvg_hip_subset_em_get(const rpvg_hip_subset_em * result, rpvg_hip_subset_em_view * view_out) {
    RPVG_REQUIRE(result && view_out, "rpvg_hip_subset_em_get: NULL argument");
    *view_out = result->view;
    view_out->num_matrices = result->num_matrices;
    return RPVG_HIP_OK;
}

extern "C" void rpvg_hip_subset_em_free(rpvg_hip_subset_em * result) { delete result; }
```

### rpvg_amd/hip.py

```python
from __future__ import annotations

import ctypes as C
import os
from typing import List, Optional, Sequence, Tuple

import numpy as np

from .batch import CClusterBatch, ClusterBatch

_HERE = os.path.dirname(os.path.abspath(__file__))
LIB_PATH = os.path.join(_HERE, "csrc", "librpvg_hip.so")

EXPORTS = [
    "rpvg_hip_device_count", "rpvg_hip_create", "rpvg_hip_create_uploader", "rpvg_hip_destroy", "rpvg_hip_last_error", "rpvg_hip_synchronize",
    "rpvg_hip_device_info", "rpvg_hip_malloc", "rpvg_hip_free", "rpvg_hip_memcpy_h2d", "rpvg_hip_memcpy_d2h",
    "rpvg_hip_batch_upload", "rpvg_hip_batch_free", "rpvg_hip_em_solve", "rpvg_hip_em_dense",
    "rpvg_hip_dense_from_cluster", "rpvg_hip_groups_build", "rpvg_hip_groups_free", "rpvg_hip_groups_collapse_info", "rpvg_hip_group_loglik",
    "rpvg_hip_synth_dense_cluster", "rpvg_hip_stats_get", "rpvg_hip_stats_reset", "rpvg_hip_stats_intervals", "rpvg_hip_em_kernel_name",
    "rpvg_hip_gibbs_read_counts", "rpvg_hip_min_path_cover", "rpvg_hip_min_path_cover_any", "rpvg_hip_cover_limits", "rpvg_hip_bounded_pair_posteriors", "rpvg_hip_pair_posteriors_get", "rpvg_hip_pair_posteriors_free",
    "rpvg_hip_em_dense_sharded", "rpvg_hip_synth_dense_rows", "rpvg_hip_synth_dense_cluster_batch", "rpvg_hip_comm_unique_id", "rpvg_hip_comm_init",
    "rpvg_hip_comm_destroy", "rpvg_hip_comm_allreduce_sum_f64", "rpvg_hip_comm_init_all", "rpvg_hip_gather", "rpvg_hip_host_register", "rpvg_hip_host_unregister", "rpvg_hip_group_conditionals",
    "rpvg_hip_group_gibbs", "rpvg_hip_group_gibbs_polyploid", "rpvg_hip_gibbs_sets_get", "rpvg_hip_gibbs_sets_free",
    "rpvg_hip_alignments_upload", "rpvg_hip_alignments_free", "rpvg_hip_read_rows_build", "rpvg_hip_read_rows_to_batch",
    "rpvg_hip_read_rows_view", "rpvg_hip_read_rows_sizes", "rpvg_hip_read_rows_free", "rpvg_hip_path_clusters", "rpvg_hip_debug_log",
    "rpvg_hip_nested_subset_em", "rpvg_hip_subset_em_get", "rpvg_hip_subset_em_free",
    "rpvg_hip_nested_full_subset_em", "rpvg_hip_subset_em_get_sets",
    "rpvg_hip_nested_independent_subset_em", "rpvg_hip_subset_em_get_independent", "rpvg_hip_independent_draws_get",
    "rpvg_hip_independent_limits", "rpvg_hip_independent_stats_get",
    "rpvg_hip_batch_cluster_totals", "rpvg_hip_batch_has_source_columns", "rpvg_hip_batch_source_columns_sizes",
    "rpvg_hip_batch_source_columns_get", "rpvg_hip_groups_build_from_sources", "rpvg_hip_groups_build_single_paths", "rpvg_hip_batch_upload_begin", "rpvg_hip_batch_upload_finish", "rpvg_hip_create_with_streams",
    "rpvg_hip_batch_upload_finish_queue", "rpvg_hip_batch_upload_finish_wait",
    "rpvg_hip_batch_upload_segments", "rpvg_hip_pinned_alloc", "rpvg_hip_pinned_free", "rpvg_hip_thread_wait_spin_us",
    "rpvg_hip_group_full_posteriors", "rpvg_hip_full_set_count",
    "rpvg_hip_frag_length_fit", "rpvg_hip_frag_length_table", "rpvg_hip_frag_length_table_get", "rpvg_hip_frag_length_table_free",
    "rpvg_hip_effective_lengths", "rpvg_hip_alignments_set_effective_lengths", "rpvg_hip_frag_length_eval",
    "rpvg_hip_align_index_create", "rpvg_hip_align_index_free", "rpvg_hip_align_index_add", "rpvg_hip_align_index_finish",
    "rpvg_hip_align_index_frag_counts", "rpvg_hip_align_index_view", "rpvg_hip_align_index_alignments",
    "rpvg_hip_path_table_upload", "rpvg_hip_path_table_free", "rpvg_hip_read_rows_to_batch_with_paths", "rpvg_hip_batch_path_group_ids",
    "rpvg_hip_name_groups_limits", "rpvg_hip_align_index_name_groups", "rpvg_hip_name_groups_view", "rpvg_hip_name_groups_free",
    "rpvg_hip_estimates_table_build", "rpvg_hip_estimates_table_tpm", "rpvg_hip_estimates_table_view", "rpvg_hip_estimates_table_limits",
    "rpvg_hip_estimates_table_free",
    "rpvg_hip_gibbs_table_build", "rpvg_hip_gibbs_table_view", "rpvg_hip_gibbs_table_rows", "rpvg_hip_gibbs_table_limits", "rpvg_hip_gibbs_table_free",
    "rpvg_hip_gibbs_read_counts_resident", "rpvg_hip_gibbs_samples_get", "rpvg_hip_gibbs_samples_free", "rpvg_hip_gibbs_table_build_resident",
    "rpvg_hip_gibbs_table_text", "rpvg_hip_estimates_table_text", "rpvg_hip_table_text_view", "rpvg_hip_table_text_get", "rpvg_hip_table_text_guards",
    "rpvg_hip_table_text_free",
    "rpvg_hip_align_index_alignments_collapsed",
    "rpvg_hip_batch_rows_sizes", "rpvg_hip_batch_rows_get",
    "rpvg_hip_segment_sort_words",
]

COMM_ID_BYTES = 128


class EngineError(RuntimeError):
    pass


class CEmProblems(C.Structure):
    _fields_ = [("num_problems", C.c_uint32), ("cluster", C.c_void_p), ("col_off", C.c_void_p), ("col_path", C.c_void_p),
                ("collapse_precision", C.c_double)]


class CEmResults(C.Structure):
    _fields_ = [("abundances", C.c_void_p), ("noise_count", C.c_void_p), ("total_count", C.c_void_p),
                ("iterations", C.c_void_p)]


class CGroupSpec(C.Structure):
    _fields_ = [("num_matrices", C.c_uint32), ("cluster", C.c_void_p), ("group_off", C.c_void_p),
                ("group_path_off", C.c_void_p), ("group_path", C.c_void_p), ("normalise", C.c_int32),
                ("collapse_precision", C.c_double)]


class CGibbsSpec(C.Structure):
    _fields_ = [("num_problems", C.c_uint32), ("group_size", C.c_uint32), ("matrix", C.c_void_p), ("num_chains", C.c_void_p),
                ("num_burn_its", C.c_void_p), ("num_gibbs_its", C.c_void_p), ("log_freq", C.c_void_p), ("num_generators", C.c_uint32),
                ("generator_problem_off", C.c_void_p), ("generator_problem", C.c_void_p), ("generator_words", C.c_void_p)]


class CGibbsSetsView(C.Structure):
    _fields_ = [("num_problems", C.c_uint32), ("group_size", C.c_uint32), ("set_off", C.POINTER(C.c_uint64)),
                ("first", C.POINTER(C.c_uint32)), ("second", C.POINTER(C.c_uint32)), ("count", C.POINTER(C.c_uint32)),
                ("words_consumed", C.POINTER(C.c_uint64)), ("generator_state", C.POINTER(C.c_uint32)), ("rounds", C.c_uint32),
                ("conditionals", C.c_uint64), ("members", C.POINTER(C.c_uint32))]


class CPairPosteriorsView(C.Structure):
    _fields_ = [("num_matrices", C.c_uint32), ("pair_off", C.POINTER(C.c_uint64)), ("first", C.POINTER(C.c_uint32)),
                ("second", C.POINTER(C.c_uint32)), ("posterior", C.POINTER(C.c_double))]


class CSubsetEmSetsView(C.Structure):
    _fields_ = [("num_matrices", C.c_uint32), ("group_size", C.c_uint32), ("subset_off", C.POINTER(C.c_uint64)),
                ("weight", C.POINTER(C.c_double)), ("path_off", C.POINTER(C.c_uint64)), ("path", C.POINTER(C.c_uint32)),
                ("col_off", C.POINTER(C.c_uint64)), ("col_path", C.POINTER(C.c_uint32)), ("abundances", C.POINTER(C.c_double)),
                ("noise_count", C.POINTER(C.c_double)), ("total_count", C.POINTER(C.c_double)), ("iterations", C.POINTER(C.c_uint32)),
                ("retained_off", C.POINTER(C.c_uint64)), ("retained_rank", C.POINTER(C.c_uint64)),
                ("retained_posterior", C.POINTER(C.c_double)), ("set_count", C.POINTER(C.c_uint32)),
                ("cluster_noise_count", C.POINTER(C.c_double)), ("set_size", C.POINTER(C.c_uint32)), ("set_member", C.POINTER(C.c_uint32)),
                ("set_posterior", C.POINTER(C.c_double)), ("set_abundance", C.POINTER(C.c_double))]


class CIndependentSpec(C.Structure):
    _fields_ = [("num_clusters", C.c_uint32), ("matrix_off", C.c_void_p), ("group_size", C.c_uint32), ("column_counts", C.c_void_p),
                ("log_freq", C.c_void_p), ("min_hap_prob", C.c_double), ("max_em_its", C.c_uint32), ("max_rel_em_conv", C.c_double),
                ("collapse_precision", C.c_double), ("generator_words", C.c_void_p), ("keep_draws", C.c_int32)]


class CSubsetEmIndependentView(C.Structure):
    _fields_ = [("num_clusters", C.c_uint32), ("group_size", C.c_uint32), ("num_samples", C.c_uint32), ("subset_off", C.POINTER(C.c_uint64)),
                ("weight", C.POINTER(C.c_double)), ("path_off", C.POINTER(C.c_uint64)), ("path", C.POINTER(C.c_uint32)),
                ("col_off", C.POINTER(C.c_uint64)), ("col_path", C.POINTER(C.c_uint32)), ("abundances", C.POINTER(C.c_double)),
                ("noise_count", C.POINTER(C.c_double)), ("total_count", C.POINTER(C.c_double)), ("iterations", C.POINTER(C.c_uint32)),
                ("set_count", C.POINTER(C.c_uint32)), ("cluster_noise_count", C.POINTER(C.c_double)), ("set_size", C.POINTER(C.c_uint32)),
                ("set_member", C.POINTER(C.c_uint32)), ("set_posterior", C.POINTER(C.c_double)), ("set_abundance", C.POINTER(C.c_double)),
                ("sample_count", C.POINTER(C.c_uint32)), ("words_consumed", C.POINTER(C.c_uint64)), ("generator_state", C.POINTER(C.c_uint32))]


class CIndependentLimits(C.Structure):
    _fields_ = [("max_group_size", C.c_uint32), ("max_samples", C.c_uint32), ("max_transcript_sets", C.c_uint64), ("words_per_draw", C.c_uint32),
                ("state_words", C.c_uint32), ("max_work_bytes", C.c_uint64)]


class CIndependentStats(C.Structure):
    _fields_ = [("calls_completed", C.c_uint64), ("draws", C.c_uint64), ("subsets", C.c_uint64)]


def independent_limits() -> CIndependentLimits:
    out = CIndependentLimits()
    lib().rpvg_hip_independent_limits(C.byref(out))
    return out


EM_KERNELS = 12


class CEmKernelStats(C.Structure):
    _fields_ = [("ms", C.c_double), ("launches", C.c_uint64), ("problems", C.c_uint64), ("iterations", C.c_uint64),
                ("max_iterations", C.c_uint64), ("alg_bytes", C.c_double)]


class CKernelStats(C.Structure):
    _fields_ = [
        ("em_sparse_ms", C.c_double), ("em_sparse_launches", C.c_uint64), ("em_sparse_alg_bytes", C.c_double),
        ("em_dense_ms", C.c_double), ("em_dense_launches", C.c_uint64), ("em_dense_alg_bytes", C.c_double),
        ("loglik_ms", C.c_double), ("loglik_launches", C.c_uint64), ("loglik_evals", C.c_double),
        ("build_ms", C.c_double), ("build_launches", C.c_uint64),
        ("h2d_ms", C.c_double), ("h2d_bytes", C.c_double),
        ("em_iterations_total", C.c_uint64),
        ("search_pairs_possible", C.c_double), ("search_pairs_table", C.c_double), ("search_pairs_kept", C.c_double),
        ("em_kernel", CEmKernelStats * EM_KERNELS),
        ("collapse_ms", C.c_double), ("busy_ms", C.c_double), ("gibbs_ms", C.c_double),
        ("search_tile_ms", C.c_double), ("search_tile_launches", C.c_uint64),
        ("gibbs_calls_completed", C.c_uint64),
        ("gibbs_count_grid_problems", C.c_uint64), ("gibbs_count_grid_iterations", C.c_uint64),
        ("cover_grid_problems", C.c_uint64), ("cover_grid_rounds", C.c_uint64),
        ("text_exact_cells", C.c_uint64),
        ("nested_full_calls", C.c_uint64), ("nested_full_sets", C.c_uint64), ("nested_full_retained", C.c_uint64),
    ]

    def as_dict(self):
        d = {n: getattr(self, n) for n, _ in self._fields_ if n != "em_kernel"}
        d["em_kernel"] = {em_kernel_name(i): {n: getattr(self.em_kernel[i], n) for n, _ in CEmKernelStats._fields_} for i in range(EM_KERNELS)}
        return d


GRID_NEVER = 2 ** 64 - 1


class CCoverLimits(C.Structure):
    _fields_ = [("workgroup_max_paths", C.c_uint32), ("chunk_rounds", C.c_uint32), ("default_grid_min_work", C.c_uint64),
                ("grid_max_rows", C.c_uint64), ("grid_max_entries", C.c_uint64), ("pick_block", C.c_uint32), ("pick_per_thread", C.c_uint32),
                ("pick_max_blocks", C.c_uint32), ("strike_block", C.c_uint32), ("strike_max_blocks", C.c_uint32), ("hist_max_paths", C.c_uint32)]


def cover_limits() -> CCoverLimits:
    out = CCoverLimits()
    lib().rpvg_hip_cover_limits(C.byref(out))
    return out


def em_kernel_name(index: int) -> str:
    f = lib().rpvg_hip_em_kernel_name
    f.restype = C.c_char_p
    return f(index).decode()


_lib = None


def lib() -> C.CDLL:
    global _lib
    if _lib is None:
        if not os.path.exists(LIB_PATH):
            raise EngineError(f"{LIB_PATH} is missing: build it with `python -c 'import __graft_entry__ as g; g.build()'` "
                              "(there is no CPU fallback)")
        L = C.CDLL(LIB_PATH)
        L.rpvg_hip_last_error.restype = C.c_char_p
        L.rpvg_hip_full_set_count.restype = C.c_uint64
        L.rpvg_hip_cover_limits.restype = None
        L.rpvg_hip_independent_limits.restype = None
        for name in EXPORTS:
            getattr(L, name)
        _lib = L
    return _lib


def _check(rc: int, what: str):
    if rc != 0:
        raise EngineError(f"{what} failed ({rc}): {lib().rpvg_hip_last_error().decode()}")


def device_count() -> int:
    n = C.c_int(0)
    rc = lib().rpvg_hip_device_count(C.byref(n))
    return n.value if rc == 0 else 0


class CClusterSegment(C.Structure):
    _fields_ = [("base", C.c_void_p), ("bytes", C.c_uint64), ("num_rows", C.c_uint32), ("num_groups", C.c_uint32), ("num_entries", C.c_uint32),
                ("num_paths", C.c_uint32), ("num_sources", C.c_uint32), ("has_paths", C.c_uint32), ("total_read_count", C.c_uint64),
                ("row_count_at", C.c_uint64), ("row_noise_at", C.c_uint64), ("row_grp_off_at", C.c_uint64), ("grp_idx_off_at", C.c_uint64),
                ("grp_prob_at", C.c_uint64), ("path_idx_at", C.c_uint64), ("path_group_id_at", C.c_uint64), ("path_source_off_at", C.c_uint64),
                ("source_id_at", C.c_uint64), ("has_columns", C.c_uint32), ("num_columns", C.c_uint32), ("num_column_paths", C.c_uint32),
                ("max_column_paths", C.c_uint32), ("col_count_at", C.c_uint64), ("col_end_at", C.c_uint64), ("col_path_at", C.c_uint64)]


class PinnedSegments:

    def __init__(self, host: ClusterBatch, with_paths: bool = True, columns=None):
        L = lib()
        L.rpvg_hip_pinned_free.argtypes = [C.c_void_p]
        K = host.num_clusters
        self.blocks = []
        self.segments = (CClusterSegment * max(K, 1))()
        self.arrays = []
        for k in range(K):
            r0, r1 = int(host.cluster_row_off[k]), int(host.cluster_row_off[k + 1])
            p0, p1 = int(host.cluster_path_off[k]), int(host.cluster_path_off[k + 1])
            g0, g1 = int(host.row_grp_off[r0]), int(host.row_grp_off[r1])
            e0, e1 = int(host.grp_idx_off[g0]), int(host.grp_idx_off[g1])
            s0, s1 = (int(host.path_source_off[p0]), int(host.path_source_off[p1])) if with_paths else (0, 0)
            pieces = [("row_noise", host.row_noise[r0:r1], np.float64), ("grp_prob", host.grp_prob[g0:g1], np.float64),
                      ("row_count", host.row_count[r0:r1], np.uint32), ("row_grp_off", host.row_grp_off[r0:r1 + 1] - g0, np.uint32),
                      ("grp_idx_off", host.grp_idx_off[g0:g1 + 1] - e0, np.uint32), ("path_idx", host.path_idx[e0:e1], np.uint32)]
            if columns is not None:
                counts, lists = columns[k]
                ends = np.cumsum([len(x) for x in lists]).astype(np.uint32) if lists else np.zeros(0, dtype=np.uint32)
                flat = np.array([p for x in lists for p in x], dtype=np.uint32)
                pieces += [("path_group_id", host.path_group_id[p0:p1], np.uint32), ("col_count", np.array(counts, dtype=np.uint32), np.uint32),
                           ("col_end", ends, np.uint32), ("col_path", flat, np.uint32)]
            elif with_paths:
# ... 145 lines not shown
        _check(lib().rpvg_hip_read_rows_to_batch_with_paths(self.ctx.handle, self.handle, index.handle, table.handle, C.byref(h)),
               "rpvg_hip_read_rows_to_batch_with_paths")
        return DeviceBatch.from_handle(self.ctx, h, K, P)

    def free(self):
        if self.handle:
            lib().rpvg_hip_read_rows_free(self.ctx.handle, self.handle)
            self.handle = C.c_void_p()

    def __del__(self):
        try:
            self.free()
        except Exception:
            pass


class DeviceAlignments:

    def __init__(self, ctx: "Context", host):
        self.ctx = ctx
        self.host = host
        self.handle = C.c_void_p()
        cb = host.as_c()
        _check(lib().rpvg_hip_alignments_upload(ctx.handle, C.byref(cb), C.byref(self.handle)), "rpvg_hip_alignments_upload")
        self.num_paths = len(host.path_effective_length)

    @classmethod
    def from_handle(cls, ctx: "Context", handle, num_paths: int) -> "DeviceAlignments":
        self = cls.__new__(cls)
        self.ctx, self.host, self.handle, self.num_paths = ctx, None, handle, num_paths
        return self

    def build_rows(self, row_params, merge: bool = True) -> DeviceRows:
        cp = row_params.as_c()
        h = C.c_void_p()
        _check(lib().rpvg_hip_read_rows_build(self.ctx.handle, self.handle, C.byref(cp), C.c_int32(1 if merge else 0), C.byref(h)),
               "rpvg_hip_read_rows_build")
        return DeviceRows(self.ctx, h)

    def set_effective_lengths(self, path_lengths, loc: float, scale: float, shape: float) -> np.ndarray:
        path_lengths = np.ascontiguousarray(path_lengths, dtype=np.uint32)
        assert path_lengths.size == self.num_paths
        out = np.zeros(path_lengths.size, dtype=np.float64)
        _check(lib().rpvg_hip_alignments_set_effective_lengths(
            self.ctx.handle, self.handle, C.c_double(loc), C.c_double(scale), C.c_double(shape),
            C.c_void_p(path_lengths.ctypes.data if path_lengths.size else None), C.c_void_p(out.ctypes.data if out.size else None)),
            "rpvg_hip_alignments_set_effective_lengths")
        return out

    def free(self):
        if self.handle:
            lib().rpvg_hip_alignments_free(self.ctx.handle, self.handle)
            self.handle = C.c_void_p()

    def __del__(self):
        try:
            self.free()
        except Exception:
            pass


class CFragLengthFit(C.Structure):
    _fields_ = [("loc", C.c_double), ("scale", C.c_double), ("shape", C.c_double), ("max_length", C.c_uint32),
                ("sample_size", C.c_uint32), ("iterations", C.c_uint32), ("evaluations", C.c_uint32), ("valid", C.c_int32)]


def frag_length_fit(ctx_handle, counts, skew_normal: bool = True) -> CFragLengthFit:
    counts = np.ascontiguousarray(counts, dtype=np.uint32)
    fit = CFragLengthFit()
    _check(lib().rpvg_hip_frag_length_fit(ctx_handle, C.c_void_p(counts.ctypes.data if counts.size else None), C.c_uint32(counts.size),
                                          C.c_int(1 if skew_normal else 0), C.byref(fit)), "rpvg_hip_frag_length_fit")
    return fit


def effective_lengths(ctx_handle, path_lengths, loc: float, scale: float, shape: float) -> np.ndarray:
    path_lengths = np.ascontiguousarray(path_lengths, dtype=np.uint32)
    out = np.zeros(path_lengths.size, dtype=np.float64)
    _check(lib().rpvg_hip_effective_lengths(ctx_handle, C.c_double(loc), C.c_double(scale), C.c_double(shape),
                                            C.c_void_p(path_lengths.ctypes.data if path_lengths.size else None),
                                            C.c_uint64(path_lengths.size), C.c_void_p(out.ctypes.data if out.size else None)),
           "rpvg_hip_effective_lengths")
    return out


class DeviceFragTable:

    def __init__(self, ctx_handle, loc: float, scale: float, shape: float):
        self.ctx_handle = ctx_handle
        self.handle = C.c_void_p()
        _check(lib().rpvg_hip_frag_length_table(ctx_handle, C.c_double(loc), C.c_double(scale), C.c_double(shape), C.byref(self.handle)),
               "rpvg_hip_frag_length_table")

    def download(self) -> np.ndarray:
        out = np.zeros(65536, dtype=np.float64)
        _check(lib().rpvg_hip_frag_length_table_get(self.ctx_handle, self.handle, C.c_void_p(out.ctypes.data)),
               "rpvg_hip_frag_length_table_get")
        return out

    def free(self):
        if self.handle:
            lib().rpvg_hip_frag_length_table_free(self.ctx_handle, self.handle)
            self.handle = C.c_void_p()

    def __del__(self):
        try:
            self.free()
        except Exception:
            pass


def host_register(array: np.ndarray):
    if array.nbytes:
        _check(lib().rpvg_hip_host_register(C.c_void_p(array.ctypes.data), C.c_uint64(array.nbytes)), "rpvg_hip_host_register")


def host_unregister(array: np.ndarray):
    if array.nbytes:
        _check(lib().rpvg_hip_host_unregister(C.c_void_p(array.ctypes.data)), "rpvg_hip_host_unregister")


class DeviceGroups:
    def __init__(self, ctx: "Context", batch: DeviceBatch, clusters: Sequence[int], groups: Sequence[Sequence[Sequence[int]]],
                 normalise: bool, collapse_precision: float = 0.0):
        self.ctx = ctx
        self.batch = batch
        cl = np.ascontiguousarray(clusters, dtype=np.uint32)
        if groups is None:
            self.handle = C.c_void_p()
            _check(lib().rpvg_hip_groups_build_single_paths(ctx.handle, batch.handle, C.c_uint32(len(cl)), C.c_void_p(cl.ctypes.data),
                                                            C.c_int32(1 if normalise else 0), C.c_double(float(collapse_precision)),
                                                            C.byref(self.handle)), "rpvg_hip_groups_build_single_paths")
            return
        goff, gpoff, gp = [0], [0], []
        for cols in groups:
            for paths in cols:
                gp.extend(paths)
                gpoff.append(len(gp))
            goff.append(len(gpoff) - 1)
        goff = np.ascontiguousarray(goff, dtype=np.uint64)
        gpoff = np.ascontiguousarray(gpoff, dtype=np.uint64)
        gp = np.ascontiguousarray(gp, dtype=np.uint32)
        spec = CGroupSpec(len(cl), cl.ctypes.data, goff.ctypes.data, gpoff.ctypes.data, gp.ctypes.data, 1 if normalise else 0,
                          float(collapse_precision))
        self.handle = C.c_void_p()
        _check(lib().rpvg_hip_groups_build(ctx.handle, batch.handle, C.byref(spec), C.byref(self.handle)),
               "rpvg_hip_groups_build")

    def collapse_info(self):
        out = [C.c_uint32(0) for _ in range(4)]
        _check(lib().rpvg_hip_groups_collapse_info(self.ctx.handle, self.handle, *[C.byref(x) for x in out]),
               "rpvg_hip_groups_collapse_info")
        return tuple(int(x.value) for x in out)

    def loglik(self, matrix, members, divisor: float, add_rowmax=None) -> np.ndarray:
        mt = np.ascontiguousarray(matrix, dtype=np.uint32)
        mem = np.ascontiguousarray(members, dtype=np.uint32)
        if mem.ndim == 1:
            mem = mem.reshape(len(mt), -1)
        width = mem.shape[1]
        out = np.zeros(len(mt), dtype=np.float64)
        flag = None if add_rowmax is None else np.ascontiguousarray(add_rowmax, dtype=np.uint8)
        _check(lib().rpvg_hip_group_loglik(self.ctx.handle, self.handle, C.c_uint32(len(mt)), C.c_void_p(mt.ctypes.data),
                                           C.c_void_p(mem.ctypes.data), C.c_uint32(width), C.c_double(divisor),
                                           C.c_void_p(flag.ctypes.data if flag is not None else None),
                                           C.c_void_p(out.ctypes.data)), "rpvg_hip_group_loglik")
        return out

    def conditionals(self, matrix, others, width: int, divisor: float, num_cols) -> List[np.ndarray]:
        mt = np.ascontiguousarray(matrix, dtype=np.uint32)
        oth = np.ascontiguousarray(others, dtype=np.uint32).reshape(len(mt), max(width - 1, 0))
        sizes = [int(num_cols[int(m)]) for m in mt]
        out = np.zeros(sum(sizes), dtype=np.float64)
        _check(lib().rpvg_hip_group_conditionals(self.ctx.handle, self.handle, C.c_uint32(len(mt)), C.c_void_p(mt.ctypes.data),
                                                 C.c_void_p(oth.ctypes.data if oth.size else None), C.c_uint32(width),
                                                 C.c_double(divisor), C.c_void_p(out.ctypes.data)),
               "rpvg_hip_group_conditionals")
        return np.split(out, np.cumsum(sizes)[:-1]) if sizes else []

    def full_posteriors(self, matrix, group_size: int, log_freq, num_cols) -> List[np.ndarray]:
        mt = np.ascontiguousarray(matrix, dtype=np.uint32)
        lf = np.ascontiguousarray(np.concatenate([np.asarray(x, dtype=np.float64) for x in log_freq]) if len(log_freq) else np.zeros(0))
        sizes = [int(lib().rpvg_hip_full_set_count(C.c_uint32(int(num_cols[int(m)])), C.c_uint32(group_size))) for m in mt]
        out = np.zeros(sum(s for s in sizes if s <= 0x7fffffff), dtype=np.float64)
        _check(lib().rpvg_hip_group_full_posteriors(self.ctx.handle, self.handle, C.c_uint32(len(mt)), C.c_void_p(mt.ctypes.data),
                                                    C.c_uint32(group_size), C.c_void_p(lf.ctypes.data if lf.size else None),
                                                    C.c_void_p(out.ctypes.data if out.size else None)),
               "rpvg_hip_group_full_posteriors")
        return np.split(out, np.cumsum(sizes)[:-1]) if sizes else []

    def nested_full_subset_em(self, group_size: int, log_freq, min_hap_prob: float, max_em_its: int = 10000, max_rel_em_conv: float = 1e-3,
                              collapse_precision: float = 0.0) -> dict:
        lf = np.ascontiguousarray(np.concatenate([np.asarray(x, dtype=np.float64) for x in log_freq]) if len(log_freq) else np.zeros(0))
        h = C.c_void_p()
        _check(lib().rpvg_hip_nested_full_subset_em(self.ctx.handle, self.batch.handle, self.handle, C.c_uint32(group_size),
                                                    C.c_void_p(lf.ctypes.data if lf.size else None), C.c_double(float(min_hap_prob)),
                                                    C.c_uint32(max_em_its), C.c_double(float(max_rel_em_conv)),
                                                    C.c_double(float(collapse_precision)), C.byref(h)), "rpvg_hip_nested_full_subset_em")
        try:
            v = CSubsetEmSetsView()
            _check(lib().rpvg_hip_subset_em_get_sets(h, C.byref(v)), "rpvg_hip_subset_em_get_sets")
            M, g = int(v.num_matrices), int(v.group_size)

            def take(pointer, n, dtype, shape=None):
                if n == 0 or not pointer:
                    return np.zeros(shape if shape is not None else (0,), dtype=dtype)
                a = np.ctypeslib.as_array(pointer, shape=(n,)).copy()
                return a.reshape(shape) if shape is not None else a

            out = {"num_matrices": M, "group_size": g}
            if M == 0:
                out.update({"subset_off": np.zeros(1, np.uint64), "path_off": np.zeros(1, np.uint64), "col_off": np.zeros(1, np.uint64),
                            "retained_off": np.zeros(1, np.uint64)})
                for name, dtype in (("weight", np.float64), ("path", np.uint32), ("col_path", np.uint32), ("abundances", np.float64),
                                    ("noise_count", np.float64), ("total_count", np.float64), ("iterations", np.uint32),
                                    ("retained_rank", np.uint64), ("retained_posterior", np.float64), ("set_count", np.uint32),
                                    ("cluster_noise_count", np.float64), ("set_size", np.uint32), ("set_posterior", np.float64)):
                    out[name] = np.zeros(0, dtype)
                out["set_member"] = np.zeros((0, g), np.uint32)
                out["set_abundance"] = np.zeros((0, g), np.float64)
                return out
            out["subset_off"] = take(v.subset_off, M + 1, np.uint64)
            S = int(out["subset_off"][-1])
            out["path_off"] = take(v.path_off, S + 1, np.uint64)
            out["col_off"] = take(v.col_off, S + 1, np.uint64)
            L, Cn = int(out["path_off"][-1]), int(out["col_off"][-1])
            out["weight"] = take(v.weight, S, np.float64)
            out["path"] = take(v.path, L, np.uint32)
            out["col_path"] = take(v.col_path, Cn, np.uint32)
            out["abundances"] = take(v.abundances, Cn, np.float64)
            out["noise_count"] = take(v.noise_count, S, np.float64)
            out["total_count"] = take(v.total_count, S, np.float64)
            out["iterations"] = take(v.iterations, S, np.uint32)
            out["retained_off"] = take(v.retained_off, M + 1, np.uint64)
            R = int(out["retained_off"][-1])
            out["retained_rank"] = take(v.retained_rank, R, np.uint64)
            out["retained_posterior"] = take(v.retained_posterior, R, np.float64)
            out["set_count"] = take(v.set_count, M, np.uint32)
            out["cluster_noise_count"] = take(v.cluster_noise_count, M, np.float64)
            out["set_size"] = take(v.set_size, L, np.uint32)
            out["set_member"] = take(v.set_member, L * g, np.uint32, (L, g))
            out["set_posterior"] = take(v.set_posterior, L, np.float64)
            out["set_abundance"] = take(v.set_abundance, L * g, np.float64, (L, g))
            return out
        finally:
            lib().rpvg_hip_subset_em_free(h)

    def nested_independent_subset_em(self, matrix_off, group_size: int, min_hap_prob: float, generator_words, column_counts=None, log_freq=None,
                                     max_em_its: int = 10000, max_rel_em_conv: float = 1e-3, collapse_precision: float = 0.0,
                                     keep_draws: bool = False) -> dict:
        mo = np.ascontiguousarray(matrix_off, dtype=np.uint32)
        K = len(mo) - 1
        gw = np.ascontiguousarray(generator_words, dtype=np.uint32).reshape(K, 624)
        cc = None if column_counts is None else np.ascontiguousarray(column_counts, dtype=np.uint32)
        lf = None
        if log_freq is not None:
            lf = np.ascontiguousarray(np.concatenate([np.asarray(x, dtype=np.float64) for x in log_freq]) if len(log_freq) else np.zeros(0))
        spec = CIndependentSpec(K, mo.ctypes.data, group_size, cc.ctypes.data if cc is not None and cc.size else None,
                                lf.ctypes.data if lf is not None and lf.size else None, float(min_hap_prob), max_em_its, float(max_rel_em_conv),
                                float(collapse_precision), gw.ctypes.data if gw.size else None, 1 if keep_draws else 0)
        h = C.c_void_p()
        _check(lib().rpvg_hip_nested_independent_subset_em(self.ctx.handle, self.batch.handle, self.handle, C.byref(spec), C.byref(h)),
               "rpvg_hip_nested_independent_subset_em")
        try:
            v = CSubsetEmIndependentView()
            _check(lib().rpvg_hip_subset_em_get_independent(h, C.byref(v)), "rpvg_hip_subset_em_get_independent")
            g = int(v.group_size)

            def take(pointer, n, dtype, shape=None):
                if n == 0 or not pointer:
                    return np.zeros(shape if shape is not None else (0,), dtype=dtype)
                a = np.ctypeslib.as_array(pointer, shape=(n,)).copy()
                return a.reshape(shape) if shape is not None else a

            out = {"num_clusters": K, "group_size": g, "num_samples": int(v.num_samples)}
            out["subset_off"] = take(v.subset_off, K + 1, np.uint64) if K else np.zeros(1, np.uint64)
            S = int(out["subset_off"][-1])
            out["path_off"] = take(v.path_off, S + 1, np.uint64) if K else np.zeros(1, np.uint64)
            out["col_off"] = take(v.col_off, S + 1, np.uint64) if K else np.zeros(1, np.uint64)
            L, Cn = int(out["path_off"][-1]), int(out["col_off"][-1])
            out["weight"] = take(v.weight, S, np.float64)
            out["path"] = take(v.path, L, np.uint32)
            out["col_path"] = take(v.col_path, Cn, np.uint32)
            out["abundances"] = take(v.abundances, Cn, np.float64)
            out["noise_count"] = take(v.noise_count, S, np.float64)
            out["total_count"] = take(v.total_count, S, np.float64)
            out["iterations"] = take(v.iterations, S, np.uint32)
            out["set_count"] = take(v.set_count, K, np.uint32)
            out["cluster_noise_count"] = take(v.cluster_noise_count, K, np.float64)
            out["set_size"] = take(v.set_size, L, np.uint32)
            out["set_member"] = take(v.set_member, L * g, np.uint32, (L, g))
            out["set_posterior"] = take(v.set_posterior, L, np.float64)
            out["set_abundance"] = take(v.set_abundance, L * g, np.float64, (L, g))
            out["sample_count"] = take(v.sample_count, S, np.uint32)
            out["words_consumed"] = take(v.words_consumed, K, np.uint64)
            out["generator_state"] = take(v.generator_state, K * 624, np.uint32, (K, 624))
            if keep_draws:
                out["draws"] = []
                for k in range(K):
                    T = int(mo[k + 1]) - int(mo[k])
                    d = np.zeros(max(out["num_samples"] * T, 1), dtype=np.uint32)
                    _check(lib().rpvg_hip_independent_draws_get(h, C.c_uint32(k), C.c_void_p(d.ctypes.data)), "rpvg_hip_independent_draws_get")
                    out["draws"].append(d[:out["num_samples"] * T].reshape(out["num_samples"], T))
            return out
        finally:
            lib().rpvg_hip_subset_em_free(h)

    def gibbs(self, matrix, group_size: int, num_chains, num_burn_its, num_gibbs_its, log_freq, generator_problems, generator_words):
        return self._gibbs("rpvg_hip_group_gibbs", matrix, group_size, num_chains, num_burn_its, num_gibbs_its, log_freq, generator_problems,
                           generator_words)

    def gibbs_polyploid(self, matrix, group_size: int, num_chains, num_burn_its, num_gibbs_its, log_freq, generator_problems, generator_words):
        return self._gibbs("rpvg_hip_group_gibbs_polyploid", matrix, group_size, num_chains, num_burn_its, num_gibbs_its, log_freq,
                           generator_problems, generator_words)

    def _gibbs(self, entry, matrix, group_size, num_chains, num_burn_its, num_gibbs_its, log_freq, generator_problems, generator_words):
        mt = np.ascontiguousarray(matrix, dtype=np.uint32)
        ch = np.ascontiguousarray(num_chains, dtype=np.uint32)
        bu = np.ascontiguousarray(num_burn_its, dtype=np.uint32)
        it = np.ascontiguousarray(num_gibbs_its, dtype=np.uint32)
        lf = np.ascontiguousarray(np.concatenate([np.asarray(x, dtype=np.float64) for x in log_freq]) if len(log_freq) else np.zeros(0))
        goff = np.ascontiguousarray(np.concatenate([[0], np.cumsum([len(g) for g in generator_problems])]), dtype=np.uint32)
        gp = np.ascontiguousarray([p for g in generator_problems for p in g], dtype=np.uint32)
        gw = np.ascontiguousarray(generator_words, dtype=np.uint32).reshape(len(generator_problems), 624)
        spec = CGibbsSpec(len(mt), group_size, mt.ctypes.data, ch.ctypes.data, bu.ctypes.data, it.ctypes.data, lf.ctypes.data,
                          len(generator_problems), goff.ctypes.data, gp.ctypes.data, gw.ctypes.data)
        h = C.c_void_p()
        _check(getattr(lib(), entry)(self.ctx.handle, self.handle, C.byref(spec), C.byref(h)), entry)
        try:
            v = CGibbsSetsView()
            _check(lib().rpvg_hip_gibbs_sets_get(h, C.byref(v)), "rpvg_hip_gibbs_sets_get")
            off = np.ctypeslib.as_array(v.set_off, shape=(len(mt) + 1,)).copy()
            total = int(off[-1])
            by_members = bool(v.members)
            if by_members:
                members = np.ctypeslib.as_array(v.members, shape=(total, group_size)).copy()
            else:
                first = np.ctypeslib.as_array(v.first, shape=(total,)).copy() if total else np.zeros(0, np.uint32)
                second = np.ctypeslib.as_array(v.second, shape=(total,)).copy() if total else np.zeros(0, np.uint32)
            count = np.ctypeslib.as_array(v.count, shape=(total,)).copy() if total else np.zeros(0, np.uint32)
            if len(generator_problems):
                words = np.ctypeslib.as_array(v.words_consumed, shape=(len(generator_problems),)).copy()
# ... 326 lines not shown
```

Measured before the change: 2.526 billion.

## Route small-matrix row partitioning and subset merging to wave-per-item kernels

Matrices with few rows are now row-partitioned by one 64-lane wave each, using ballot/popcount counting with no LDS or block barriers. Larger matrices keep the 1024-thread block kernel through an item list. The subset merge step similarly splits clusters between wave-sized and workgroup roles, and a debug row-readback API plus Python bindings are added. This targets the waste of launching 1024-thread blocks with heavy syncing for tiny matrices, at the cost of extra item-list uploads and two launches.

```diff
diff --git a/include/rpvg_hip.h b/include/rpvg_hip.h
--- a/include/rpvg_hip.h
+++ b/include/rpvg_hip.h
@@ -417,6 +417,9 @@
 
 int rpvg_hip_debug_log(rpvg_hip_ctx * ctx, uint64_t n, const double * x, double * out, int32_t use_table);
 
+int rpvg_hip_debug_group_rows(rpvg_hip_ctx * ctx, const rpvg_hip_groups * groups, uint32_t * row_perm_out, uint32_t * mat_fast_out,
+                              uint32_t * mat_mid_out);
+
 #define RPVG_HIP_EM_KERNELS 12
 typedef struct rpvg_hip_em_kernel_stats {
     double ms;
diff --git a/rpvg_amd/csrc/group_build.hip b/rpvg_amd/csrc/group_build.hip
--- a/rpvg_amd/csrc/group_build.hip
+++ b/rpvg_amd/csrc/group_build.hip
@@ -18,14 +18,14 @@
 
 template <int BLOCK>
 __global__ __launch_bounds__(BLOCK) void partitionRowsKernel(
-    const uint32_t num_matrices, const uint64_t * __restrict__ mat_row_off, const uint64_t * __restrict__ mat_row0,
+    const uint32_t num_items, const uint32_t * __restrict__ item_matrix, const uint64_t * __restrict__ mat_row_off, const uint64_t * __restrict__ mat_row0,
     const uint64_t * __restrict__ mat_rows, const double * __restrict__ row_count, const double * __restrict__ row_noise,
     uint32_t * __restrict__ row_perm, double * __restrict__ count_out, double * __restrict__ noise_out,
     uint32_t * __restrict__ mat_fast, uint32_t * __restrict__ mat_mid, const uint32_t mid_min_rows) {
     __shared__ uint32_t class_base[kNumRowClasses];
     __shared__ uint32_t wave_count[BLOCK / 64][kNumRowClasses];
-    const uint32_t m = blockIdx.x;
-    if (m >= num_matrices) return;
+    if (blockIdx.x >= num_items) return;
+    const uint32_t m = item_matrix ? item_matrix[blockIdx.x] : blockIdx.x;
     const uint32_t R = static_cast<uint32_t>(mat_rows[m]);
     const double * cnt = row_count + mat_row0[m];
     const double * nz = row_noise + mat_row0[m];
@@ -73,6 +73,76 @@
             class_base[threadIdx.x] += added;
         }
         __syncthreads();
+    }
+}
+
+constexpr uint32_t kPartitionAhead = 4;
+
+__global__ __launch_bounds__(kPartitionWaveThreads) void partitionRowsWaveKernel(
+    const uint32_t num_items, const uint32_t * __restrict__ item_matrix, const uint64_t * __restrict__ mat_row_off, const uint64_t * __restrict__ mat_row0,
+    const uint64_t * __restrict__ mat_rows, const double * __restrict__ row_count, const double * __restrict__ row_noise,
+    uint32_t * __restrict__ row_perm, double * __restrict__ count_out, double * __restrict__ noise_out,
+    uint32_t * __restrict__ mat_fast, uint32_t * __restrict__ mat_mid, const uint32_t mid_min_rows) {
+    const uint32_t lane = threadIdx.x & 63u;
+    const uint32_t item = __builtin_amdgcn_readfirstlane(blockIdx.x * (kPartitionWaveThreads / 64) + (threadIdx.x >> 6));
+    if (item >= num_items) return;
+    const uint32_t m = item_matrix[item];
+    const uint64_t R = mat_rows[m];
+    const double * cnt = row_count + mat_row0[m];
+    const double * nz = row_noise + mat_row0[m];
+    const uint64_t out0 = mat_row_off[m];
+    const bool with_mid = R >= mid_min_rows;
+    const unsigned long long below = (1ull << lane) - 1ull;
+    uint32_t base[kNumRowClasses];
+#pragma unroll
+    for (uint32_t k = 0; k < kNumRowClasses; ++k) base[k] = 0;
+    for (uint64_t c0 = 0; c0 < R; c0 += 64 * kPartitionAhead) {
+        uint32_t mine[kPartitionAhead];
+#pragma unroll
+        for (uint32_t u = 0; u < kPartitionAhead; ++u) {
+            const uint64_t i = c0 + 64 * u + lane;
+            mine[u] = i < R ? rowClass(cnt[i], nz[i], with_mid) : kNumRowClasses;
+        }
+#pragma unroll
+        for (uint32_t u = 0; u < kPartitionAhead; ++u) {
+#pragma unroll
+            for (uint32_t k = 0; k < kNumRowClasses; ++k) base[k] += __popcll(__ballot(mine[u] == k));
+        }
+    }
+    uint32_t running = 0;
+#pragma unroll
+    for (uint32_t k = 0; k < kNumRowClasses; ++k) {
+        const uint32_t n = base[k];
+        base[k] = running;
+        running += n;
+        if (k == 0 && lane == 0) mat_fast[m] = running;
+        if (k + 2 == kNumRowClasses && lane == 0) mat_mid[m] = running;
+    }
+    for (uint64_t c0 = 0; c0 < R; c0 += 64 * kPartitionAhead) {
+        double c[kPartitionAhead], z[kPartitionAhead];
+#pragma unroll
+        for (uint32_t u = 0; u < kPartitionAhead; ++u) {
+            const uint64_t i = c0 + 64 * u + lane;
+            c[u] = i < R ? cnt[i] : 0.0;
+            z[u] = i < R ? nz[i] : 0.0;
+        }
+#pragma unroll
+        for (uint32_t u = 0; u < kPartitionAhead; ++u) {
+            const uint64_t i = c0 + 64 * u + lane;
+            const uint32_t mine = i < R ? rowClass(c[u], z[u], with_mid) : kNumRowClasses;
+            uint32_t dest = 0;
+#pragma unroll
+            for (uint32_t k = 0; k < kNumRowClasses; ++k) {
+                const unsigned long long ballot = __ballot(mine == k);
+                if (mine == k) dest = base[k] + __popcll(ballot & below);
+                base[k] += __popcll(ballot);
+            }
+            if (i < R) {
+                row_perm[out0 + dest] = static_cast<uint32_t>(i);
+                count_out[out0 + dest] = c[u];
+                noise_out[out0 + dest] = z[u];
+            }
+        }
     }
 }
 
@@ -692,6 +762,7 @@
     DeviceBuffer<uint64_t> inc_off, path_grp_off, group_off, group_path_off, num_paths;
     DeviceBuffer<uint32_t> path_grp, group_path, degree, cursor, cluster;
     ItemBuffers list_items, tile_items, mask_items, word_items;
+    DeviceBuffer<uint32_t> partition_wave_matrix, partition_block_matrix;
     DeviceBuffer<uint64_t> mask_off, masks, first_path, word_off, path_words;
     DeviceBuffer<uint32_t> column_counts;
     DeviceBuffer<unsigned char> scan_tmp;
@@ -721,6 +792,13 @@
     knobs.masks = masks_env ? std::atoi(masks_env) != 0 : true;
     knobs.words = masks_env ? std::atoi(masks_env) >= 2 : true;
     knobs.direct = !std::getenv("RPVG_HIP_NO_DIRECT_BUILD");
+    static const uint32_t partition_wave_rows = [] {
+        const char * per_matrix = std::getenv("RPVG_HIP_PARTITION_PER_MATRIX");
+        if (per_matrix && std::atoi(per_matrix) != 0) return 0u;
+        const char * edge = RPVG_EXPERIMENT_ENV("RPVG_HIP_PARTITION_WAVE_ROWS");
+        return edge ? static_cast<uint32_t>(std::max(0, std::atoi(edge))) : kPartitionWaveMaxRows;
+    }();
+    knobs.partition_wave_rows = partition_wave_rows;
     return knobs;
 }
 
@@ -760,6 +838,8 @@
         pack.addZero(t.path_words, p.word_total);
     }
     pack.add(t.cluster, s.spec->cluster, M);
+    if (!p.partition_wave_matrix.empty()) pack.add(t.partition_wave_matrix, p.partition_wave_matrix.data(), p.partition_wave_matrix.size());
+    if (!p.partition_block_matrix.empty()) pack.add(t.partition_block_matrix, p.partition_block_matrix.data(), p.partition_block_matrix.size());
     if (p.lists_needed) {
         pack.addZero(t.degree, p.inc_total);
         pack.addZero(t.cursor, p.inc_total);
@@ -835,9 +915,15 @@
 void queuePartition(BuildState & s) {
     const GroupBuildPlan & p = s.plan;
     rpvg_hip_groups * g = s.g;
-    partitionRowsKernel<kPartitionThreads><<<dim3(p.partition.grid), dim3(p.partition.block), 0, s.st>>>(
-        p.M, g->mat_row_off.ptr, g->mat_row0.ptr, g->mat_rows.ptr, s.batch->row_count.ptr, s.batch->row_noise.ptr, g->row_perm.ptr, g->row_count.ptr,
-        g->row_noise.ptr, g->mat_fast.ptr, g->mat_mid.ptr, kMidMinRows);
+    const auto launch = [&](auto kernel, const Launch & l, const size_t matrices, const uint32_t * item_matrix) {
+        if (l.grid == 0) return;
+        kernel<<<dim3(l.grid), dim3(l.block), 0, s.st>>>(static_cast<uint32_t>(matrices), item_matrix, g->mat_row_off.ptr, g->mat_row0.ptr, g->mat_rows.ptr,
+                                                         s.batch->row_count.ptr, s.batch->row_noise.ptr, g->row_perm.ptr, g->row_count.ptr, g->row_noise.ptr,
+                                                         g->mat_fast.ptr, g->mat_mid.ptr, kMidMinRows);
+    };
+    launch(partitionRowsKernel<kPartitionThreads>, p.partition, p.partition_routes ? p.partition_block_matrix.size() : p.M,
+           p.partition_routes ? s.tmp.partition_block_matrix.ptr : nullptr);
+    launch(partitionRowsWaveKernel, p.partition_waves, p.partition_wave_matrix.size(), s.tmp.partition_wave_matrix.ptr);
 }
 
 MaskBuildArgs waveKernelArgs(const BuildState & s, const ItemBuffers & items, const uint64_t * set_off, const uint64_t * sets) {
@@ -1085,6 +1171,25 @@
     });
 }
 
+extern "C" int rpvg_hip_debug_group_rows(rpvg_hip_ctx * ctx, const rpvg_hip_groups * groups, uint32_t * row_perm_out, uint32_t * mat_fast_out,
+                                         uint32_t * mat_mid_out) {
+    RPVG_REQUIRE(ctx && groups, "rpvg_hip_debug_group_rows: NULL argument");
+    RPVG_REQUIRE(groups->num_matrices == 0 || (row_perm_out && mat_fast_out && mat_mid_out), "rpvg_hip_debug_group_rows: NULL output");
+    if (groups->num_matrices == 0) return RPVG_HIP_OK;
+    std::lock_guard<std::mutex> lock(ctx->mutex);
+    hipError_t e = hipSetDevice(ctx->device);
+    if (e == hipSuccess) e = hipStreamSynchronize(ctx->stream);
+    if (e == hipSuccess) e = hipMemcpyAsync(row_perm_out, groups->row_perm.ptr, groups->row_perm.count * sizeof(uint32_t), hipMemcpyDeviceToHost, ctx->stream);
+    if (e == hipSuccess) e = hipMemcpyAsync(mat_fast_out, groups->mat_fast.ptr, groups->num_matrices * sizeof(uint32_t), hipMemcpyDeviceToHost, ctx->stream);
+    if (e == hipSuccess) e = hipMemcpyAsync(mat_mid_out, groups->mat_mid.ptr, groups->num_matrices * sizeof(uint32_t), hipMemcpyDeviceToHost, ctx->stream);
+    if (e == hipSuccess) e = hipStreamSynchronize(ctx->stream);
+    if (e != hipSuccess) {
+        setError("rpvg_hip_debug_group_rows: %s", hipGetErrorString(e));
+        return RPVG_HIP_ERR_RUNTIME;
+    }
+    return RPVG_HIP_OK;
+}
+
 int rpvg_hip_groups::buildError(hipStream_t stream) const {
     if (build_checked || !build_error_flag.ptr) return RPVG_HIP_OK;
     uint32_t bad = 0;
diff --git a/rpvg_amd/csrc/group_build_plan.hpp b/rpvg_amd/csrc/group_build_plan.hpp
--- a/rpvg_amd/csrc/group_build_plan.hpp
+++ b/rpvg_amd/csrc/group_build_plan.hpp
@@ -35,6 +35,8 @@
 
 constexpr uint32_t kTileLdsBytes = (kTileDoubles + 256) * sizeof(double);
 constexpr uint32_t kPartitionThreads = 1024;
+constexpr uint32_t kPartitionWaveThreads = 256;
+constexpr uint32_t kPartitionWaveMaxRows = 1024;
 
 constexpr uint32_t kCollapseMaxMatrices = 1u << 20;
 constexpr int kStatusOk = 0, kStatusInvalid = -3;
@@ -49,6 +51,7 @@
     bool masks = true;
     bool words = true;
     bool direct = true;
+    uint32_t partition_wave_rows = 0;
 };
 
 struct Launch {
@@ -76,12 +79,14 @@
     std::vector<uint32_t> cols, max_col_paths, paths, cluster;
     uint64_t val_total = 0, row_total = 0, inc_total = 0, mask_total = 0, word_total = 0;
     Items list_items, tile_items, mask_items, word_items;
+    std::vector<uint32_t> partition_wave_matrix, partition_block_matrix;
+    bool partition_routes = false;
     bool lists_needed = false;
     bool direct = false;
     uint64_t num_columns = 0, num_incidences = 0;
     double h2d_bytes = 0;
     Launch gather_columns, single_path_columns;
-    Launch zero_wide, partition;
+    Launch zero_wide, partition, partition_waves;
     Launch build_single_paths, column_masks, build_masks;
     Launch path_words, build_words;
     Launch incidence_count, incidence_fill;
@@ -138,6 +143,7 @@
         p.val_total += R * (g1 - g0);
         p.row_total += R;
         p.inc_total += N + 1;
+        if (knobs.partition_wave_rows > 0) (R <= knobs.partition_wave_rows ? p.partition_wave_matrix : p.partition_block_matrix).push_back(m);
         const uint64_t mask_words = (N + 63) / 64;
         if (p.direct) {
             p.mask_items.add(m, R, kMaskRows);
@@ -163,7 +169,8 @@
     if (M == 0) return p;
     p.num_columns = group_off[M];
     p.num_incidences = kind == Columns::Lists ? group_path_off[p.num_columns] : group_path_off[M];
-    p.h2d_bytes = static_cast<double>(M * 60 + p.num_columns * 8 + p.num_incidences * 4 + (p.list_items.size() + p.tile_items.size()) * 8);
+    p.h2d_bytes = static_cast<double>(M * 60 + p.num_columns * 8 + p.num_incidences * 4 + (p.list_items.size() + p.tile_items.size()) * 8 +
+                                      (p.partition_wave_matrix.size() + p.partition_block_matrix.size()) * 4);
 
     const auto items = [](const Items & list) { return static_cast<uint32_t>(list.size()); };
     const auto waves = [](const Items & list) { return list.empty() ? Launch{} : Launch{(static_cast<uint32_t>(list.size()) + 3) / 4, 256, 0}; };
@@ -172,7 +179,15 @@
     if (kind == Columns::Sources) p.gather_columns = per_matrix;
     if (kind == Columns::SinglePaths) p.single_path_columns = per_matrix;
     if (!p.list_items.empty()) p.zero_wide = p.build_lists = Launch{items(p.list_items), kListRows, 0};
-    p.partition = Launch{M, kPartitionThreads, 0};
+    p.partition_routes = knobs.partition_wave_rows > 0;
+    if (!p.partition_routes) {
+        p.partition = Launch{M, kPartitionThreads, 0};
+    } else {
+        constexpr uint32_t per_block = kPartitionWaveThreads / 64;
+        const uint32_t waves_n = static_cast<uint32_t>(p.partition_wave_matrix.size()), blocks_n = static_cast<uint32_t>(p.partition_block_matrix.size());
+        if (waves_n) p.partition_waves = Launch{(waves_n + per_block - 1) / per_block, kPartitionWaveThreads, 0};
+        if (blocks_n) p.partition = Launch{blocks_n, kPartitionThreads, 0};
+    }
     if (p.direct) {
         p.build_single_paths = waves(p.mask_items);
     } else if (!p.mask_items.empty()) {
diff --git a/rpvg_amd/csrc/subset_em.hip b/rpvg_amd/csrc/subset_em.hip
--- a/rpvg_amd/csrc/subset_em.hip
+++ b/rpvg_amd/csrc/subset_em.hip
@@ -359,23 +359,84 @@
     unsigned char * packed;
 };
 
-__global__ __launch_bounds__(256) void subsetMergeKernel(const MergeArgs args) {
+struct MergeOutputs {
+    uint32_t * set_count;
+    double * cluster_noise;
+    uint32_t * set_first;
+    uint32_t * set_second;
+    double * set_posterior;
+    double * set_abund;
+};
+
+__device__ __forceinline__ MergeOutputs mergeOutputs(const MergeArgs & args, const SubsetHeader & h) {
+    const PackedLayout lay = packedLayout(args.num_matrices, h.subsets, h.list_length, h.columns);
+    return {reinterpret_cast<uint32_t *>(args.packed + lay.set_count), reinterpret_cast<double *>(args.packed + lay.cluster_noise),
+            reinterpret_cast<uint32_t *>(args.packed + lay.set_first), reinterpret_cast<uint32_t *>(args.packed + lay.set_second),
+            reinterpret_cast<double *>(args.packed + lay.set_posterior), reinterpret_cast<double *>(args.packed + lay.set_abund)};
+}
+
+__device__ __forceinline__ unsigned long long mergeRecord(const MergeArgs & args, const uint64_t s0, const uint32_t n, const uint64_t base,
+                                                          const uint32_t * __restrict__ gid, const uint32_t pos, double & a0, double & a1) {
+    uint32_t lo = 0, hi = n - 1;
+    while (lo < hi) {
+        const uint32_t mid = (lo + hi + 1) >> 1;
+        if (args.path_off[s0 + mid] - base <= pos) lo = mid; else hi = mid - 1;
+    }
+    const uint32_t r = lo;
+    const uint32_t l0 = static_cast<uint32_t>(args.path_off[s0 + r] - base), L = static_cast<uint32_t>(args.path_off[s0 + r + 1] - base) - l0;
+    const uint32_t * list = args.path + base + l0;
+    const uint32_t j = pos - l0;
+    const uint32_t g = gid[list[j]];
+    uint32_t members = 0, first = 0, second = 0;
+    for (uint32_t t = 0; t < L; ++t) {
+        if (gid[list[t]] == g) {
+            if (members == 0) first = t;
+            else if (members == 1) second = t;
+            ++members;
+        }
+    }
+    if (members > 2) *args.merge_bad = 1;
+    if (first != j || members > 2) return kMergeNoRecord;
+    const uint32_t p0 = list[first], p1 = (members == 2) ? list[second] : 0xffffffffu;
+    const double w = args.weight[s0 + r];
+    const uint64_t c0 = args.col_off[s0 + r];
+    const uint32_t C = static_cast<uint32_t>(args.col_off[s0 + r + 1] - c0);
+    const uint32_t * cols = args.col_path + c0;
+    auto column = [&](const uint32_t p) {
+        uint32_t a = 0, b = C;
+        while (a < b) {
+            const uint32_t mid = (a + b) >> 1;
+            if (cols[mid] < p) a = mid + 1; else b = mid;
+        }
+        return a;
+    };
+    const double multiplicity = (members == 2 && p0 == p1) ? 2.0 : 1.0;
+    a0 = mulRounded(args.abundances[c0 + column(p0)], w) / multiplicity;
+    a1 = (members == 2) ? mulRounded(args.abundances[c0 + column(p1)], w) / multiplicity : 0.0;
+    return (static_cast<unsigned long long>(p0 + 1) << (kMergePathBits + kMergeRankBits)) |
+           (static_cast<unsigned long long>(members == 2 ? p1 + 1 : 0u) << kMergeRankBits) | r;
+}
+
+__device__ __forceinline__ double mergeNoiseCount(const MergeArgs & args, const uint64_t s0, const uint32_t n) {
+    double noise = 0.0, sum_hap_prob = 0.0;
+    for (uint32_t r = 0; r < n; ++r) {
+        const double w = args.weight[s0 + r];
+        sum_hap_prob = addRounded(sum_hap_prob, w);
+        noise = addRounded(noise, mulRounded(args.noise[s0 + r], w));
+    }
+    return addRounded(noise, mulRounded(addRounded(1.0, -sum_hap_prob), args.total[s0]));
+}
+
+__device__ __forceinline__ void mergeClusterByWorkgroup(const MergeArgs & args, const MergeOutputs & out, const uint32_t m, unsigned long long * s_key,
+                                                        uint32_t * s_pos, uint32_t * s_scan) {
     constexpr int BLOCK = 256;
-    __shared__ unsigned long long s_key[kMergeLdsRecords];
-    __shared__ uint32_t s_pos[kMergeLdsRecords];
-    __shared__ uint32_t s_scan[BLOCK / 64];
-    const SubsetHeader h = *args.header;
-    if (h.overflow) return;
-    const uint32_t m = blockIdx.x, tid = threadIdx.x;
-    const uint64_t M = args.num_matrices;
-    if (m >= M) return;
-    const PackedLayout lay = packedLayout(M, h.subsets, h.list_length, h.columns);
-    uint32_t * set_count = reinterpret_cast<uint32_t *>(args.packed + lay.set_count);
-    double * cluster_noise = reinterpret_cast<double *>(args.packed + lay.cluster_noise);
-    uint32_t * set_first = reinterpret_cast<uint32_t *>(args.packed + lay.set_first);
-    uint32_t * set_second = reinterpret_cast<uint32_t *>(args.packed + lay.set_second);
-    double * set_posterior = reinterpret_cast<double *>(args.packed + lay.set_posterior);
-    double * set_abund = reinterpret_cast<double *>(args.packed + lay.set_abund);
+    const uint32_t tid = threadIdx.x;
+    uint32_t * const set_count = out.set_count;
+    double * const cluster_noise = out.cluster_noise;
+    uint32_t * const set_first = out.set_first;
+    uint32_t * const set_second = out.set_second;
+    double * const set_posterior = out.set_posterior;
+    double * const set_abund = out.set_abund;
     const uint64_t s0 = args.subset_off[m];
     const uint32_t n = static_cast<uint32_t>(args.subset_off[m + 1] - s0);
     if (n == 0) {
@@ -388,15 +449,7 @@
     const uint64_t base = args.path_off[s0];
     const uint32_t Lm = static_cast<uint32_t>(args.path_off[s0 + n] - base);
     const uint32_t * gid = args.path_group_id + args.cluster_path_off[args.cluster[m]];
-    if (tid == BLOCK - 1) {
-        double noise = 0.0, sum_hap_prob = 0.0;
-        for (uint32_t r = 0; r < n; ++r) {
-            const double w = args.weight[s0 + r];
-            sum_hap_prob = addRounded(sum_hap_prob, w);
-            noise = addRounded(noise, mulRounded(args.noise[s0 + r], w));
-        }
-        cluster_noise[m] = addRounded(noise, mulRounded(addRounded(1.0, -sum_hap_prob), args.total[s0]));
-    }
+    if (tid == BLOCK - 1) cluster_noise[m] = mergeNoiseCount(args, s0, n);
     uint32_t P2 = 2;
     while (P2 < Lm) P2 <<= 1;
     unsigned long long * keys = s_key;
@@ -408,44 +461,11 @@
     for (uint32_t pos = tid; pos < P2; pos += BLOCK) {
         unsigned long long key = kMergeNoRecord;
         if (pos < Lm) {
-            uint32_t lo = 0, hi = n - 1;
-            while (lo < hi) {
-                const uint32_t mid = (lo + hi + 1) >> 1;
-                if (args.path_off[s0 + mid] - base <= pos) lo = mid; else hi = mid - 1;
-            }
-            const uint32_t r = lo;
-            const uint32_t l0 = static_cast<uint32_t>(args.path_off[s0 + r] - base), L = static_cast<uint32_t>(args.path_off[s0 + r + 1] - base) - l0;
-            const uint32_t * list = args.path + base + l0;
-            const uint32_t j = pos - l0;
-            const uint32_t g = gid[list[j]];
-            uint32_t members = 0, first = 0, second = 0;
-            for (uint32_t t = 0; t < L; ++t) {
-                if (gid[list[t]] == g) {
-                    if (members == 0) first = t;
-                    else if (members == 1) second = t;
-                    ++members;
-                }
-            }
-            if (members > 2) *args.merge_bad = 1;
-            if (first == j && members <= 2) {
-                const uint32_t p0 = list[first], p1 = (members == 2) ? list[second] : 0xffffffffu;
-                const double w = args.weight[s0 + r];
-                const uint64_t c0 = args.col_off[s0 + r];
-                const uint32_t C = static_cast<uint32_t>(args.col_off[s0 + r + 1] - c0);
-                const uint32_t * cols = args.col_path + c0;
-                auto column = [&](const uint32_t p) {
-                    uint32_t a = 0, b = C;
-                    while (a < b) {
-                        const uint32_t mid = (a + b) >> 1;
-                        if (cols[mid] < p) a = mid + 1; else b = mid;
-                    }
-                    return a;
-                };
-                const double multiplicity = (members == 2 && p0 == p1) ? 2.0 : 1.0;
-                args.rec_a0[base + pos] = mulRounded(args.abundances[c0 + column(p0)], w) / multiplicity;
-                args.rec_a1[base + pos] = (members == 2) ? mulRounded(args.abundances[c0 + column(p1)], w) / multiplicity : 0.0;
-                key = (static_cast<unsigned long long>(p0 + 1) << (kMergePathBits + kMergeRankBits)) |
-                      (static_cast<unsigned long long>(members == 2 ? p1 + 1 : 0u) << kMergeRankBits) | r;
+            double a0 = 0.0, a1 = 0.0;
+            key = mergeRecord(args, s0, n, base, gid, pos, a0, a1);
+            if (key != kMergeNoRecord) {
+                args.rec_a0[base + pos] = a0;
+                args.rec_a1[base + pos] = a1;
             }
         }
         keys[pos] = key;
@@ -499,7 +519,182 @@
     if (tid == 0) set_count[m] = Q;
 }
 
-}
+__global__ __launch_bounds__(256) void subsetMergeKernel(const MergeArgs args) {
+    __shared__ unsigned long long s_key[kMergeLdsRecords];
+    __shared__ uint32_t s_pos[kMergeLdsRecords];
+    __shared__ uint32_t s_scan[256 / 64];
+    const SubsetHeader h = *args.header;
+    if (h.overflow) return;
+    if (blockIdx.x >= args.num_matrices) return;
+    mergeClusterByWorkgroup(args, mergeOutputs(args, h), blockIdx.x, s_key, s_pos, s_scan);
+}
+
+constexpr uint32_t kMergeWaveRecords = 64;
+constexpr uint32_t kMergeGroupBlocks = 128;
+constexpr uint32_t kMergeScanClusters = 64;
+
+struct MergeRoles {
+    uint32_t wave_blocks, group_blocks;
+    uint32_t wave_records;
+};
+
+__device__ __forceinline__ unsigned long long laneValue(const unsigned long long v, const uint32_t uniform_lane) {
+    const uint32_t lo = __builtin_amdgcn_readlane(static_cast<int>(static_cast<uint32_t>(v)), uniform_lane);
+    const uint32_t hi = __builtin_amdgcn_readlane(static_cast<int>(static_cast<uint32_t>(v >> 32)), uniform_lane);
+    return (static_cast<unsigned long long>(hi) << 32) | lo;
+}
+
+__device__ __forceinline__ bool mergeClusterByWave(const MergeArgs & args, const MergeOutputs & out, const uint32_t m, const uint32_t wave_records) {
+    const uint32_t lane = threadIdx.x & 63u;
+    const uint64_t s0 = args.subset_off[m];
+    const uint32_t n = __builtin_amdgcn_readfirstlane(static_cast<uint32_t>(args.subset_off[m + 1] - s0));
+    if (n == 0) {
+        if (lane == 0) {
+            out.set_count[m] = 0;
+            out.cluster_noise[m] = 0.0;
+        }
+        return true;
+    }
+    const uint64_t base = args.path_off[s0];
+    const uint64_t length = args.path_off[s0 + n] - base;
+    if (length > wave_records) return false;
+    const uint32_t Lm = __builtin_amdgcn_readfirstlane(static_cast<uint32_t>(length));
+    const uint32_t * gid = args.path_group_id + args.cluster_path_off[args.cluster[m]];
+    if (lane == 63) out.cluster_noise[m] = mergeNoiseCount(args, s0, n);
+
+    unsigned long long key = kMergeNoRecord;
+    double a0 = 0.0, a1 = 0.0, weight = 0.0;
+    if (lane < Lm) {
+        key = mergeRecord(args, s0, n, base, gid, lane, a0, a1);
+        if (key != kMergeNoRecord) weight = args.weight[s0 + static_cast<uint32_t>(key & ((1u << kMergeRankBits) - 1u))];
+    }
+    uint32_t rank = lane < Lm ? 0u : lane;
+    for (uint32_t i = 0; i < Lm; ++i) {
+        const unsigned long long other = laneValue(key, i);
+        if (lane < Lm && (other < key || (other == key && i < lane))) ++rank;
+    }
+    uint32_t source = lane;
+    for (uint32_t i = 0; i < Lm; ++i) {
+        if (static_cast<uint32_t>(__builtin_amdgcn_readlane(static_cast<int>(rank), i)) == lane) source = i;
+    }
+    key = __shfl(key, static_cast<int>(source));
+    a0 = __shfl(a0, static_cast<int>(source));
+    a1 = __shfl(a1, static_cast<int>(source));
+    weight = __shfl(weight, static_cast<int>(source));
+
+    const unsigned long long set = key >> kMergeRankBits;
+    const unsigned long long set_before = __shfl_up(set, 1);
+    const bool start = key != kMergeNoRecord && (lane == 0 || set_before != set);
+    const unsigned long long starts = __ballot(start);
+    double posterior = 0.0, sum0 = 0.0, sum1 = 0.0;
+    bool going = start;
+    for (uint32_t t = 0; __ballot(going) != 0ull; ++t) {
+        const int from = static_cast<int>((lane + t) & 63u);
+        const unsigned long long their_key = __shfl(key, from);
+        const double their_weight = __shfl(weight, from), their_a0 = __shfl(a0, from), their_a1 = __shfl(a1, from);
+        going = going && lane + t < 64 && their_key != kMergeNoRecord && (their_key >> kMergeRankBits) == set;
+        if (going) {
+            posterior = addRounded(posterior, their_weight);
+            sum0 = addRounded(sum0, their_a0);
+            sum1 = addRounded(sum1, their_a1);
+        }
+    }
+    if (start) {
+        const uint64_t q = base + __popcll(starts & ((1ull << lane) - 1ull));
+        const uint32_t second = static_cast<uint32_t>(set & ((1u << kMergePathBits) - 1u));
+        out.set_first[q] = static_cast<uint32_t>(set >> kMergePathBits) - 1;
+        out.set_second[q] = second ? second - 1 : 0xffffffffu;
+        out.set_posterior[q] = posterior;
+        out.set_abund[2 * q] = sum0;
+        out.set_abund[2 * q + 1] = sum1;
+    }
+    if (lane == 0) out.set_count[m] = __popcll(starts);
+    return true;
+}
+
+__global__ __launch_bounds__(256) void subsetMergeRolesKernel(const MergeArgs args, const MergeRoles roles) {
+    __shared__ unsigned long long s_key[kMergeLdsRecords];
+    __shared__ uint32_t s_pos[kMergeLdsRecords];
+    __shared__ uint32_t s_scan[256 / 64];
+    __shared__ uint32_t s_long[kMergeScanClusters + 1];
+    const SubsetHeader h = *args.header;
+    if (h.overflow) return;
+    const uint32_t M = args.num_matrices;
+    const MergeOutputs out = mergeOutputs(args, h);
+    if (blockIdx.x >= roles.group_blocks) {
+        const uint32_t m = __builtin_amdgcn_readfirstlane((blockIdx.x - roles.group_blocks) * 4 + (threadIdx.x >> 6));
+        if (m < M) (void) mergeClusterByWave(args, out, m, roles.wave_records);
+        return;
+    }
+    const uint32_t b = blockIdx.x;
+    for (uint64_t first = b; first < M; first += static_cast<uint64_t>(kMergeScanClusters) * roles.group_blocks) {
+        if (threadIdx.x < 64) {
+            const uint64_t m = first + static_cast<uint64_t>(threadIdx.x) * roles.group_blocks;
+            bool is_long = false;
+            if (threadIdx.x < kMergeScanClusters && m < M) {
+                const uint64_t s0 = args.subset_off[m], s1 = args.subset_off[m + 1];
+                is_long = s1 > s0 && args.path_off[s1] - args.path_off[s0] > roles.wave_records;
+            }
+            const unsigned long long all = __ballot(is_long);
+            if (is_long) s_long[__popcll(all & ((1ull << threadIdx.x) - 1ull))] = static_cast<uint32_t>(m);
+            if (threadIdx.x == 0) s_long[kMergeScanClusters] = __popcll(all);
+        }
+        __syncthreads();
+        const uint32_t count = s_long[kMergeScanClusters];
+        for (uint32_t k = 0; k < count; ++k) {
+            mergeClusterByWorkgroup(args, out, s_long[k], s_key, s_pos, s_scan);
+            __syncthreads();
+        }
+        __syncthreads();
+    }
+}
+
+}
+
+static MergeRoles mergeRoles(const uint32_t M) {
+    static const bool per_cluster = [] {
+        const char * env = std::getenv("RPVG_HIP_MERGE_PER_CLUSTER");
+        return env != nullptr && std::atoi(env) != 0;
+    }();
+    static const uint32_t wave_records = [] {
+        const char * env = RPVG_EXPERIMENT_ENV("RPVG_HIP_MERGE_WAVE_RECORDS");
+        return env ? static_cast<uint32_t>(std::min(std::max(std::atoi(env), 0), static_cast<int>(kMergeWaveRecords))) : kMergeWaveRecords;
+    }();
+    static const uint32_t group_blocks = [] {
+        const char * env = RPVG_EXPERIMENT_ENV("RPVG_HIP_MERGE_GROUP_BLOCKS");
+        return env ? static_cast<uint32_t>(std::min(std::max(std::atoi(env), 1), 4096)) : kMergeGroupBlocks;
+    }();
+    if (per_cluster || M == 0) return {0, 0, 0};
+    return {(M + 3) / 4, std::min(group_blocks, M), wave_records};
+}
+
+#ifdef RPVG_HIP_EXPERIMENTS
+static void printMergeHistogram(hipStream_t st, const SubsetHeader * d_header, const uint32_t M, const uint64_t * d_subset_off, const uint64_t * d_path_off) {
+    static bool printed = false;
+    if (printed) return;
+    printed = true;
+    SubsetHeader h;
+    if (hipStreamSynchronize(st) != hipSuccess || hipMemcpy(&h, d_header, sizeof(h), hipMemcpyDeviceToHost) != hipSuccess || h.overflow) return;
+    std::vector<uint64_t> subset_off(M + 1), path_off(h.subsets + 1);
+    if (hipMemcpy(subset_off.data(), d_subset_off, subset_off.size() * 8, hipMemcpyDeviceToHost) != hipSuccess ||
+        hipMemcpy(path_off.data(), d_path_off, path_off.size() * 8, hipMemcpyDeviceToHost) != hipSuccess) return;
+    const uint32_t edges[] = {0, 8, 16, 32, 64, 128, 256, 512, 1024, 2048};
+    std::vector<uint64_t> bins(sizeof(edges) / sizeof(edges[0]) + 1, 0);
+    uint64_t longest = 0;
+    for (uint32_t m = 0; m < M; ++m) {
+        const uint64_t L = path_off[subset_off[m + 1]] - path_off[subset_off[m]];
+        longest = std::max(longest, L);
+        size_t b = 0;
+        while (b < sizeof(edges) / sizeof(edges[0]) && L > edges[b]) ++b;
+        ++bins[b];
+    }
+    std::fprintf(stderr, "[rpvg_hip merge histogram] %u clusters, %llu subsets, longest list %llu; lists of", M, h.subsets, static_cast<unsigned long long>(longest));
+    for (size_t b = 0; b < bins.size(); ++b) {
+        if (b < sizeof(edges) / sizeof(edges[0])) std::fprintf(stderr, " <=%u: %llu", edges[b], static_cast<unsigned long long>(bins[b]));
+        else std::fprintf(stderr, " more: %llu\n", static_cast<unsigned long long>(bins[b]));
+    }
+}
+#endif
 
 
 static int nestedSubsetEmAttempt(rpvg_hip_ctx * ctx, const rpvg_hip_batch * batch, const rpvg_hip_groups * groups,
@@ -796,8 +991,13 @@
         ma.merge_bad = d_merge_bad;
         ma.packed = d_packed.ptr;
         const int merge_span = ctx->spanBegin(FAM_BUILD);
-        subsetMergeKernel<<<dim3(M), dim3(256), 0, st>>>(ma);
+        const MergeRoles roles = mergeRoles(M);
+        if (roles.wave_blocks == 0) subsetMergeKernel<<<dim3(M), dim3(256), 0, st>>>(ma);
+        else subsetMergeRolesKernel<<<dim3(roles.wave_blocks + roles.group_blocks), dim3(256), 0, st>>>(ma, roles);
         ctx->spanEnd(merge_span);
+#ifdef RPVG_HIP_EXPERIMENTS
+        if (RPVG_EXPERIMENT_ENV("RPVG_HIP_MERGE_HISTOGRAM")) printMergeHistogram(st, header, M, d_subset_off.ptr, d_path_off.ptr);
+#endif
         ctx->stats.build_launches += 1;
     }
     PackArgs pa;
diff --git a/rpvg_amd/hip.py b/rpvg_amd/hip.py
--- a/rpvg_amd/hip.py
+++ b/rpvg_amd/hip.py
@@ -23,6 +23,7 @@
     "rpvg_hip_group_gibbs", "rpvg_hip_group_gibbs_polyploid", "rpvg_hip_gibbs_sets_get", "rpvg_hip_gibbs_sets_free",
     "rpvg_hip_alignments_upload", "rpvg_hip_alignments_free", "rpvg_hip_read_rows_build", "rpvg_hip_read_rows_to_batch",
     "rpvg_hip_read_rows_view", "rpvg_hip_read_rows_sizes", "rpvg_hip_read_rows_free", "rpvg_hip_path_clusters", "rpvg_hip_debug_log",
+    "rpvg_hip_debug_group_rows",
     "rpvg_hip_nested_subset_em", "rpvg_hip_subset_em_get", "rpvg_hip_subset_em_free",
     "rpvg_hip_nested_full_subset_em", "rpvg_hip_subset_em_get_sets",
     "rpvg_hip_nested_independent_subset_em", "rpvg_hip_subset_em_get_independent", "rpvg_hip_independent_draws_get",
@@ -98,6 +99,15 @@
                 ("retained_off", C.POINTER(C.c_uint64)), ("retained_rank", C.POINTER(C.c_uint64)),
                 ("retained_posterior", C.POINTER(C.c_double)), ("set_count", C.POINTER(C.c_uint32)),
                 ("cluster_noise_count", C.POINTER(C.c_double)), ("set_size", C.POINTER(C.c_uint32)), ("set_member", C.POINTER(C.c_uint32)),
+                ("set_posterior", C.POINTER(C.c_double)), ("set_abundance", C.POINTER(C.c_double))]
+
+
+class CSubsetEmView(C.Structure):
+    _fields_ = [("num_matrices", C.c_uint32), ("subset_off", C.POINTER(C.c_uint64)), ("weight", C.POINTER(C.c_double)),
+                ("path_off", C.POINTER(C.c_uint64)), ("path", C.POINTER(C.c_uint32)), ("col_off", C.POINTER(C.c_uint64)),
+                ("col_path", C.POINTER(C.c_uint32)), ("abundances", C.POINTER(C.c_double)), ("noise_count", C.POINTER(C.c_double)),
+                ("total_count", C.POINTER(C.c_double)), ("iterations", C.POINTER(C.c_uint32)), ("set_count", C.POINTER(C.c_uint32)),
+                ("cluster_noise_count", C.POINTER(C.c_double)), ("set_first", C.POINTER(C.c_uint32)), ("set_second", C.POINTER(C.c_uint32)),
                 ("set_posterior", C.POINTER(C.c_double)), ("set_abundance", C.POINTER(C.c_double))]
 
 
@@ -549,6 +559,14 @@
                "rpvg_hip_groups_collapse_info")
         return tuple(int(x.value) for x in out)
 
+    def debug_rows(self, num_matrices: int, total_rows: int):
+        perm = np.zeros(max(int(total_rows), 1), dtype=np.uint32)
+        fast = np.zeros(max(int(num_matrices), 1), dtype=np.uint32)
+        mid = np.zeros(max(int(num_matrices), 1), dtype=np.uint32)
+        _check(lib().rpvg_hip_debug_group_rows(self.ctx.handle, self.handle, C.c_void_p(perm.ctypes.data), C.c_void_p(fast.ctypes.data),
+                                               C.c_void_p(mid.ctypes.data)), "rpvg_hip_debug_group_rows")
+        return perm[:int(total_rows)], fast[:int(num_matrices)], mid[:int(num_matrices)]
+
     def loglik(self, matrix, members, divisor: float, add_rowmax=None) -> np.ndarray:
         mt = np.ascontiguousarray(matrix, dtype=np.uint32)
         mem = np.ascontiguousarray(members, dtype=np.uint32)
@@ -584,6 +602,43 @@
                                                     C.c_void_p(out.ctypes.data if out.size else None)),
                "rpvg_hip_group_full_posteriors")
         return np.split(out, np.cumsum(sizes)[:-1]) if sizes else []
+
+    def nested_subset_em(self, column_counts, min_hap_prob: float, max_em_its: int = 10000, max_rel_em_conv: float = 1e-3,
+                         collapse_precision: float = 0.0) -> dict:
+        counts = np.ascontiguousarray(column_counts, dtype=np.uint32)
+        h = C.c_void_p()
+        _check(lib().rpvg_hip_nested_subset_em(self.ctx.handle, self.batch.handle, self.handle, C.c_void_p(counts.ctypes.data if counts.size else None),
+                                               C.c_double(float(min_hap_prob)), C.c_double(float(min_hap_prob)), C.c_uint32(max_em_its),
+                                               C.c_double(float(max_rel_em_conv)), C.c_double(float(collapse_precision)), C.byref(h)),
+               "rpvg_hip_nested_subset_em")
+        try:
+            v = CSubsetEmView()
+            _check(lib().rpvg_hip_subset_em_get(h, C.byref(v)), "rpvg_hip_subset_em_get")
+            M = int(v.num_matrices)
+
+            def take(pointer, n, dtype, shape=None):
+                if n == 0 or not pointer:
+                    return np.zeros(shape if shape is not None else (0,), dtype=dtype)
+                a = np.ctypeslib.as_array(pointer, shape=(n,)).copy()
+                return a.reshape(shape) if shape is not None else a
+
+            out = {"num_matrices": M}
+            out["subset_off"] = take(v.subset_off, M + 1, np.uint64) if M else np.zeros(1, np.uint64)
+            S = int(out["subset_off"][-1])
+            out["path_off"] = take(v.path_off, S + 1, np.uint64) if M else np.zeros(1, np.uint64)
+            out["col_off"] = take(v.col_off, S + 1, np.uint64) if M else np.zeros(1, np.uint64)
+            L, Cn = int(out["path_off"][-1]), int(out["col_off"][-1])
+            for name, pointer, n, dtype in (("weight", v.weight, S, np.float64), ("path", v.path, L, np.uint32), ("col_path", v.col_path, Cn, np.uint32),
+                                            ("abundances", v.abundances, Cn, np.float64), ("noise_count", v.noise_count, S, np.float64),
+                                            ("total_count", v.total_count, S, np.float64), ("iterations", v.iterations, S, np.uint32),
+                                            ("set_count", v.set_count, M, np.uint32), ("cluster_noise_count", v.cluster_noise_count, M, np.float64),
+                                            ("set_first", v.set_first, L, np.uint32), ("set_second", v.set_second, L, np.uint32),
+                                            ("set_posterior", v.set_posterior, L, np.float64)):
+                out[name] = take(pointer, n, dtype)
+            out["set_abundance"] = take(v.set_abundance, 2 * L, np.float64, (L, 2))
+            return out
+        finally:
+            lib().rpvg_hip_subset_em_free(h)
 
     def nested_full_subset_em(self, group_size: int, log_freq, min_hap_prob: float, max_em_its: int = 10000, max_rel_em_conv: float = 1e-3,
                               collapse_precision: float = 0.0) -> dict:
```

After: 2.536 billion, median of 3. About the same (+0.4%).
